# verdurin/pbdagcon

Hardware: AMD Instinct MI355X
Metric: consensus bases/sec (whole node) (higher is better)
Workload: dtype u8

## Files before the change

### pbdagcon_amd/csrc/dagcon_api.hip

```cpp
#include <hip/hip_runtime.h>
#include <algorithm>
#include <cstdarg>
#include <cstdio>
#include <cstdlib>
#include <cstring>
#include <string>
#include <chrono>
#include <vector>

#include "../../include/dagcon.h"
#include "dagcon_dev.h"
#include "k_build.hip.h"
#include "k_merge.hip.h"
#include "k_merge_q.hip.h"
#include "k_bestpath.hip.h"
#include "k_align.hip.h"
#include "k_align_panels.hip.h"
#include "k_place.hip.h"
#include "k_cigar.hip.h"
#include "k_cs.hip.h"

namespace {

struct DevBuf {
    void *p = nullptr;
    size_t cap = 0;
};

#define DQ_KMAX 52u
struct DgPlanIn { uint32_t T; uint64_t n_alns, sum_bb; uint32_t gcuts, max_segments, min_segment_len, seg_env, merge_q; };
struct DgPlan { uint32_t seg_max, seg_min, use_q, bp_max; };
static DgPlan dg_plan_pieces(const DgPlanIn &in) {
    DgPlan pl;
    const uint32_t T = in.T;
    pl.seg_min = in.min_segment_len;
    if (!pl.seg_min) pl.seg_min = (uint32_t)std::min<uint64_t>(768, std::max<uint64_t>(192, in.sum_bb / 8192));
    if (in.max_segments) pl.seg_max = in.max_segments > 64u ? 64u : in.max_segments;
    else if (in.seg_env) pl.seg_max = in.seg_env;
    else if (in.gcuts) pl.seg_max = 64;
    else { uint32_t sm = T ? 8192u / T : 8u; pl.seg_max = sm < 8u ? 8u : sm > 256u ? 256u : sm; }
    if (in.gcuts && !in.min_segment_len) pl.seg_min = 256;
    pl.use_q = 0;
    if (in.merge_q && !in.gcuts && pl.seg_max != 1) {
        const uint32_t slots = 1024u * DQ_WAVES;
        if (in.max_segments || in.seg_env) pl.use_q = 1;
        else if (T && in.n_alns <= (uint64_t)DQ_KMAX * T) {
            const uint64_t avail = std::min<uint64_t>(256, std::max<uint64_t>(1, in.sum_bb / T / 128));
            const uint64_t k = (uint64_t)T * avail / DQ_ROWS / slots;
            if (k >= 1 || (uint64_t)T * avail / DQ_ROWS * 10u >= 6u * slots) {
                const uint64_t sm = std::min<uint64_t>(avail, std::max<uint64_t>(k, 1) * slots * DQ_ROWS / T);
                if (sm >= 2) { pl.seg_max = (uint32_t)sm; pl.use_q = 1; }
            }
        }
    }
    if (pl.seg_max < 1) pl.seg_max = 1;
    if (pl.use_q && !in.min_segment_len) pl.seg_min = 128;
    pl.bp_max = pl.seg_max == 1 ? 1u : std::min(in.gcuts || T >= 256u ? 64u : (uint32_t)DG_BP_PIECES, 3u * pl.seg_max);
    if (pl.bp_max < 1) pl.bp_max = 1;
    return pl;
}

struct Ctx {
    dagcon_opts opts;
    int device = 0;
    hipStream_t stream = nullptr;
    hipEvent_t ev[5] = {nullptr, nullptr, nullptr, nullptr, nullptr};
    std::string err;
    bool uploaded = false, ran = false, fetched = false;

    uint32_t T = 0, A = 0;
    int bp_lane = 1, bl_stk = -1;
    uint32_t align_dropped = 0;
    uint32_t align_n = 0;
    std::vector<uint32_t> h_ends;
    int poison = 0;
    int fold = 1;
    int merge_q = 1, use_q = 0;
    uint32_t max_k = 0, max_tlen = 0;
    uint64_t sum_len = 0, sum_bb = 0, mat_cells = 0, blob_bytes = 0;
    bool have_bb = false;
    std::vector<uint32_t> h_tlen, h_aln_len, h_aln_start, h_aln_tgt;
    std::vector<uint64_t> h_aln_begin, h_aln_off, h_mat_base, h_bbv_base, h_bb_off, h_matc_base;
    std::vector<uint32_t> h_matc_stride;
    uint64_t matc_cells = 0;
    std::vector<uint8_t> h_tactive;
    std::vector<uint32_t> h_ch_base, h_ch_aln;
    std::vector<uint64_t> h_norm_off;
    std::vector<uint32_t> h_ck_base;
    uint64_t n_ckpt = 0;
    uint32_t emit_shift = 9;
    uint32_t n_chunks = 0;
    uint64_t tmp_main = 0, tmp_cap = 0;

    DevBuf d_tfail, d_q, d_t, d_aln_off, d_aln_len, d_aln_start, d_aln_tgt, d_tlen, d_aln_begin, d_tactive,
        d_bb, d_bb_off, d_mat_base, d_bbv_base, d_matc_base, d_matc_stride;
    DevBuf d_nmis, d_norm_off, d_n_lo, d_n_hi, d_n_start, d_n_ins, d_n_del, d_norm;
    DevBuf d_ch_aln, d_ch_base, d_ch_k0, d_ch_next, d_ch_w, d_ch_tb, d_ch_flag, d_ch_src, d_ch_out, d_ch_adv,
        d_n_lb, d_norm_tmp, d_ckpt, d_ck_base;
    DevBuf d_node_base, d_n_nodes, d_pool_base, d_pool_size, d_pool_top, d_t_nins;
    DevBuf d_matA, d_matD, d_matC, d_cov, d_gcount, d_gbase, d_bid;
    DevBuf d_nodes, d_best, d_queue, d_score, d_cns_tmp, d_bp_tt, d_score_b;
    DevBuf d_pool, d_stk, d_cuts, d_cuts_bp, d_bp_stat, d_bp_len, d_worklist, d_rd, d_pro_state, d_sh_cnt, d_seg_done, d_wl_first, d_queue0, d_bp_end, d_bp_ab, d_defer, d_cns_tmp0;
    DevBuf d_al[15];
    DevBuf d_pn[18];
    DevBuf d_pl[14];
    DevBuf d_cs[10];
    DevBuf d_cg[18];
    std::vector<uint8_t> h_cig_bad;
    std::string cig_err;
    DevBuf d_cns, d_cns_off, d_cns_len, d_seg_first, d_n_seg, d_seg_r0, d_seg_r1, d_st;
    DevBuf d_pos_tmp, d_pos_tmp0, d_pos;
    DevBuf d_sup_tmp, d_sup_tmp0, d_sup;

    uint64_t norm_cap = 0, node_cap = 0, pool_cap = 0, cns_cap = 0, seg_cap = 0;
    uint32_t stk_words = 4096, growth_pct = 100, seg_max = 8, bp_max = 16, seg_env = 0, seg_min = 768;
    uint32_t sh_log = 16;
    bool full_span = false;
    uint32_t gcuts = 1;
    uint32_t worklist_cap = 0, list_grid = 8192;

    DgStatus h_st;
    dagcon_timings tm;

    std::vector<uint64_t> r_seg_begin, r_seq_off, r_cns_off, r_seg_first;
    std::vector<int32_t> r_range0, r_range1, r_tmp0, r_tmp1;
    std::vector<uint32_t> r_seq_len, r_cns_len, r_n_seg, r_tfail;
    std::vector<int32_t> r_status;
    char *r_blob = nullptr;
    size_t r_blob_cap = 0;
    uint16_t *r_sup = nullptr;
    size_t r_sup_cap = 0;
    uint64_t r_sup_n = 0;
    std::vector<uint32_t> r_pos;
    bool pos_valid = false;
    bool sup_valid = false;

    std::vector<uint8_t> g_base, g_deleted, g_backbone;
    std::vector<int32_t> g_weight, g_cov, g_bbpos, g_out_dst, g_out_cnt, g_in_src;
    std::vector<uint32_t> g_out_begin, g_in_begin;
};

int fail(Ctx *c, int code, const char *fmt, ...) {
    char buf[512];
    va_list ap;
    va_start(ap, fmt);
    vsnprintf(buf, sizeof buf, fmt, ap);
    va_end(ap);
    if (c) c->err = buf;
    return code;
}

#define HIPCHK(c, call)                                                                    \
    do {                                                                                   \
        hipError_t _e = (call);                                                            \
        if (_e != hipSuccess)                                                              \
            return fail((c), DAGCON_ERR_HIP, "%s failed: %s (%s:%d)", #call,               \
                        hipGetErrorString(_e), __FILE__, __LINE__);                        \
    } while (0)

int ensure(Ctx *c, DevBuf &b, size_t bytes) {
    if (bytes == 0) bytes = 16;
    if (b.cap >= bytes) return DAGCON_OK;
    if (b.p) { (void)hipFree(b.p); b.p = nullptr; b.cap = 0; }
    size_t want = bytes + bytes / 16 + 256;
    const bool dbg = getenv("DAGCON_ALLOC_TIMING") != nullptr;
    const double t0 = dbg ? std::chrono::duration<double>(std::chrono::steady_clock::now().time_since_epoch()).count() : 0;
    hipError_t e = hipMalloc(&b.p, want);
    if (dbg) {
        const double dt = std::chrono::duration<double>(std::chrono::steady_clock::now().time_since_epoch()).count() - t0;
        if (dt > 0.005) fprintf(stderr, "dagcon: hipMalloc(%.1f MB) took %.1f ms\n", want / 1e6, dt * 1e3);
    }
    if (e != hipSuccess) {
        b.p = nullptr;
        return fail(c, DAGCON_ERR_WORKSPACE, "hipMalloc(%zu bytes) failed: %s", want, hipGetErrorString(e));
    }
    b.cap = want;
    return DAGCON_OK;
}

#define ENSURE(c, buf, bytes)                                \
    do {                                                     \
        int _r = ensure((c), (buf), (size_t)(bytes));        \
        if (_r != DAGCON_OK) return _r;                      \
    } while (0)

template <typename T>
int upload_vec(Ctx *c, DevBuf &b, const std::vector<T> &v) {
    ENSURE(c, b, v.size() * sizeof(T));
    if (!v.empty()) HIPCHK(c, hipMemcpyAsync(b.p, v.data(), v.size() * sizeof(T), hipMemcpyHostToDevice, c->stream));
    return DAGCON_OK;
}

void free_buf(DevBuf &b) {
    if (b.p) (void)hipFree(b.p);
    b.p = nullptr; b.cap = 0;
}

int ensure_arenas(Ctx *c) {
    ENSURE(c, c->d_norm, c->norm_cap * sizeof(uint16_t));
    ENSURE(c, c->d_nodes, c->node_cap * sizeof(DgNode));
    ENSURE(c, c->d_best, c->node_cap * 4);
    ENSURE(c, c->d_queue, c->node_cap * 4);
    ENSURE(c, c->d_score, c->node_cap * 8);
    ENSURE(c, c->d_bp_tt, c->node_cap * 4);
    if (c->gcuts) ENSURE(c, c->d_score_b, c->node_cap * 4);
    ENSURE(c, c->d_cns_tmp, c->node_cap);
    ENSURE(c, c->d_pool, c->pool_cap * 4);
    ENSURE(c, c->d_stk, std::max<uint64_t>((uint64_t)c->T * std::max(c->bp_max, c->seg_max), c->gcuts ? c->list_grid : 0) * c->stk_words * 4);
    if (c->gcuts) {
        ENSURE(c, c->d_worklist, (4ull + 3ull * c->worklist_cap) * 4);
        ENSURE(c, c->d_rd, (uint64_t)c->A * 16 + 16);
        ENSURE(c, c->d_pro_state, (uint64_t)c->T * 16 + 16);
        ENSURE(c, c->d_sh_cnt, (uint64_t)c->T * (2 + 2 * DG_SH_MAX) * 4 + 16);
        ENSURE(c, c->d_seg_done, (uint64_t)c->worklist_cap * (DG_SH_MAX + 1) * 4 + 16);
        ENSURE(c, c->d_wl_first, (uint64_t)c->T * 4 + 16);
        ENSURE(c, c->d_queue0, c->node_cap * 4);
        ENSURE(c, c->d_bp_end, (uint64_t)c->T * c->bp_max * 4 + 16);
        ENSURE(c, c->d_bp_ab, (uint64_t)c->T * c->bp_max * 16 + 16);
        ENSURE(c, c->d_defer, (uint64_t)c->T * (DG_DEFER_MAX + 1) * 4 + 16);
        ENSURE(c, c->d_cns_tmp0, c->node_cap);
    }
    ENSURE(c, c->d_cuts, (uint64_t)c->T * (c->seg_max + 2) * 4);
    ENSURE(c, c->d_cuts_bp, (uint64_t)c->T * (c->bp_max + 2) * 4);
    ENSURE(c, c->d_bp_stat, (uint64_t)c->T * c->bp_max * 8);
    ENSURE(c, c->d_bp_len, (uint64_t)c->T * c->bp_max * 4);
    ENSURE(c, c->d_cns, c->cns_cap);
    if (c->opts.flags & DAGCON_FLAG_BASE_SUPPORT) {
        ENSURE(c, c->d_sup_tmp, c->node_cap * 4);
        if (c->gcuts) ENSURE(c, c->d_sup_tmp0, c->node_cap * 4);
        ENSURE(c, c->d_sup, c->cns_cap * 4);
    }
    if (c->opts.flags & DAGCON_FLAG_BASE_POS) {
        ENSURE(c, c->d_pos_tmp, c->node_cap * 4);
        if (c->gcuts) ENSURE(c, c->d_pos_tmp0, c->node_cap * 4);
        ENSURE(c, c->d_pos, c->cns_cap * 4);
    }
    ENSURE(c, c->d_seg_r0, c->seg_cap * 4);
    ENSURE(c, c->d_seg_r1, c->seg_cap * 4);
    return DAGCON_OK;
}

void fill_params(Ctx *c, DgParams &p) {
    memset(&p, 0, sizeof p);
    p.q = (const uint8_t *)c->d_q.p; p.t = (const uint8_t *)c->d_t.p;
    p.aln_off = (const uint64_t *)c->d_aln_off.p;
    p.aln_len = (const uint32_t *)c->d_aln_len.p;
    p.aln_start = (const uint32_t *)c->d_aln_start.p;
    p.aln_tgt = (const uint32_t *)c->d_aln_tgt.p;
    p.tlen = (const uint32_t *)c->d_tlen.p;
    p.aln_begin = (const uint64_t *)c->d_aln_begin.p;
    p.tactive = (const uint8_t *)c->d_tactive.p; p.tfail = (uint32_t *)c->d_tfail.p;
    p.bb = c->have_bb ? (const uint8_t *)c->d_bb.p : nullptr;
    p.bb_off = (const uint64_t *)c->d_bb_off.p;
    p.mat_base = (const uint64_t *)c->d_mat_base.p;
    p.matc_base = (const uint64_t *)c->d_matc_base.p; p.matc_stride = (const uint32_t *)c->d_matc_stride.p;
    p.bbv_base = (const uint64_t *)c->d_bbv_base.p;
    p.T = c->T; p.A = c->A;
    p.trim = c->opts.trim; p.min_len = c->opts.min_len;
    p.min_weight = c->opts.min_weight < 0 ? (int32_t)c->opts.min_cov : c->opts.min_weight;
    p.flags = c->opts.flags;
    p.max_k = c->max_k; p.max_tlen = c->max_tlen;
    p.nmis = (uint32_t *)c->d_nmis.p; p.norm_off = (uint64_t *)c->d_norm_off.p;
    p.n_lo = (uint32_t *)c->d_n_lo.p; p.n_hi = (uint32_t *)c->d_n_hi.p;
    p.n_start = (uint32_t *)c->d_n_start.p; p.n_ins = (uint32_t *)c->d_n_ins.p;
    p.n_del = (uint32_t *)c->d_n_del.p;
    p.norm = (uint16_t *)c->d_norm.p; p.norm_cap = c->norm_cap;
    p.ch_aln = (const uint32_t *)c->d_ch_aln.p; p.ch_base = (const uint32_t *)c->d_ch_base.p;
    p.n_chunks = c->n_chunks;
    p.ch_k0 = (uint32_t *)c->d_ch_k0.p; p.ch_next = (uint32_t *)c->d_ch_next.p;
    p.ch_w = (uint32_t *)c->d_ch_w.p; p.ch_tb = (uint32_t *)c->d_ch_tb.p;
    p.ch_flag = (uint32_t *)c->d_ch_flag.p; p.ch_src = (uint64_t *)c->d_ch_src.p;
    p.ch_out = (uint32_t *)c->d_ch_out.p; p.ch_adv = (uint32_t *)c->d_ch_adv.p;
    p.n_lb = (uint32_t *)c->d_n_lb.p; p.norm_tmp = (uint16_t *)c->d_norm_tmp.p;
    p.tmp_main = c->tmp_main; p.tmp_cap = c->tmp_cap;
    p.ckpt = (uint32_t *)c->d_ckpt.p; p.ck_base = (const uint32_t *)c->d_ck_base.p; p.emit_shift = c->emit_shift;
    p.node_base = (uint64_t *)c->d_node_base.p; p.n_nodes = (uint32_t *)c->d_n_nodes.p;
    p.pool_base = (uint64_t *)c->d_pool_base.p; p.pool_size = (uint32_t *)c->d_pool_size.p;
    p.pool_top = (uint32_t *)c->d_pool_top.p; p.t_nins = (uint32_t *)c->d_t_nins.p;
    p.matA = (uint32_t *)c->d_matA.p; p.matD = (uint32_t *)c->d_matD.p; p.matC = (uint32_t *)c->d_matC.p;
    p.cov = (int32_t *)c->d_cov.p; p.gcount = (uint32_t *)c->d_gcount.p;
    p.gbase = (uint32_t *)c->d_gbase.p; p.bid = (uint32_t *)c->d_bid.p;
    p.nodes = (DgNode *)c->d_nodes.p; p.best = (int32_t *)c->d_best.p;
    p.queue = (int32_t *)c->d_queue.p; p.score = (float2 *)c->d_score.p; p.bp_tt = (float *)c->d_bp_tt.p;
    p.cns_tmp = (uint8_t *)c->d_cns_tmp.p; p.node_cap = c->node_cap;
    p.pool = (uint32_t *)c->d_pool.p; p.pool_cap = c->pool_cap;
    p.stk = (int32_t *)c->d_stk.p; p.stk_words = c->stk_words; p.growth_pct = c->growth_pct;
    p.score_b = (float *)c->d_score_b.p;
    p.bp_lane = c->bp_lane >= 2 || (c->bp_lane && (uint64_t)c->T * c->bp_max >= 32768ull) ? 1u : 0u; p.bl_stk = c->bl_stk >= 0 && c->bl_stk < DG_BL_STK ? (uint32_t)c->bl_stk : (uint32_t)DG_BL_STK;
    p.emit_scan = c->max_k <= 64u ? 1u : 0u;
    p.fold = (c->fold && !(c->opts.flags & DAGCON_FLAG_STOP_AFTER_BUILD)) ? 1u : 0u;
    p.q_kmax = c->use_q && !c->opts.max_segments && !c->seg_env && c->max_k > DQ_KMAX ? DQ_KMAX : 0u;
    p.bp_seg_min = (c->seg_min + 2u) / 3u;
    p.seg_max = c->seg_max; p.seg_min = c->seg_min; p.cuts = (uint32_t *)c->d_cuts.p; p.bp_max = c->bp_max; p.cuts_bp = (uint32_t *)c->d_cuts_bp.p; p.bp_stat = (float *)c->d_bp_stat.p; p.bp_len = (uint32_t *)c->d_bp_len.p;
    p.gcuts = c->gcuts; p.sh_log = c->sh_log;
    p.rd_s = (uint32_t *)c->d_rd.p; p.rd_e = p.rd_s + c->A; p.rd_lead = p.rd_e + c->A; p.rd_trail = p.rd_lead + c->A;
    p.pro_state = (uint32_t *)c->d_pro_state.p; p.sh_cnt = (uint32_t *)c->d_sh_cnt.p;
    p.queue0 = (int32_t *)c->d_queue0.p; p.bp_end = (uint32_t *)c->d_bp_end.p; p.bp_ab = (float *)c->d_bp_ab.p;
    p.defer = (uint32_t *)c->d_defer.p; p.cns_tmp0 = (uint8_t *)c->d_cns_tmp0.p;
    p.seg_done = (uint32_t *)c->d_seg_done.p; p.wl_first = (uint32_t *)c->d_wl_first.p;
    p.worklist = (uint32_t *)c->d_worklist.p; p.worklist_cap = c->worklist_cap;
    p.cns = (uint8_t *)c->d_cns.p; p.cns_cap = c->cns_cap;
    p.cns_off = (uint64_t *)c->d_cns_off.p; p.cns_len = (uint32_t *)c->d_cns_len.p;
    p.seg_first = (uint64_t *)c->d_seg_first.p; p.n_seg = (uint32_t *)c->d_n_seg.p;
    p.seg_r0 = (int32_t *)c->d_seg_r0.p; p.seg_r1 = (int32_t *)c->d_seg_r1.p;
    p.seg_cap = c->seg_cap;
    p.st = (DgStatus *)c->d_st.p;
    if (c->opts.flags & DAGCON_FLAG_BASE_SUPPORT) {
        p.sup_tmp = (uint32_t *)c->d_sup_tmp.p; p.sup_tmp0 = (uint32_t *)c->d_sup_tmp0.p;
        p.sup_w = (uint16_t *)c->d_sup.p; p.sup_d = p.sup_w + c->cns_cap;
    }
    if (c->opts.flags & DAGCON_FLAG_BASE_POS) {
        p.pos_tmp = (uint32_t *)c->d_pos_tmp.p; p.pos_tmp0 = (uint32_t *)c->d_pos_tmp0.p; p.pos_out = (uint32_t *)c->d_pos.p;
    }
}

void launch_normalize(Ctx *c, const DgParams &p) {
    hipStream_t s = c->stream;
    if (c->A == 0) return;
    (void)hipMemsetAsync(c->d_ckpt.p, 0xFF, c->n_ckpt * 4, s);
    hipLaunchKernelGGL((k_norm_chunk<DG_NW, 64, false>), dim3((c->n_chunks + 63) / 64), dim3(64), 0, s, p);
    hipLaunchKernelGGL((k_norm_chunk<DG_NW_BIG, 32, true>), dim3((c->n_chunks + 31) / 32), dim3(32), 0, s, p);
    hipLaunchKernelGGL(k_norm_scan, dim3((c->A + 63) / 64), dim3(64), 0, s, p);
    hipLaunchKernelGGL(k_norm_finish2, dim3((c->n_chunks + 3) / 4), dim3(256), 0, s, p);
    hipLaunchKernelGGL(k_normalize_slow, dim3((c->A + 63) / 64), dim3(64), 0, s, p);
}

int launch_all(Ctx *c) {
    int r = ensure_arenas(c);
    if (r != DAGCON_OK) return r;
    DgParams p;
    fill_params(c, p);
    hipStream_t s = c->stream;
    if (c->poison & 8) {
        DevBuf *work[] = {&c->d_nmis, &c->d_n_lo, &c->d_n_hi, &c->d_n_start, &c->d_n_ins, &c->d_n_del, &c->d_ch_k0, &c->d_ch_next, &c->d_ch_w,
                          &c->d_ch_tb, &c->d_ch_flag, &c->d_ch_src, &c->d_ch_out, &c->d_ch_adv, &c->d_n_lb, &c->d_norm_tmp, &c->d_ckpt,
                          &c->d_node_base, &c->d_n_nodes, &c->d_pool_base, &c->d_pool_size, &c->d_pool_top, &c->d_t_nins, &c->d_cov, &c->d_gcount,
                          &c->d_gbase, &c->d_bid, &c->d_best, &c->d_queue, &c->d_score, &c->d_cns_tmp, &c->d_bp_tt, &c->d_stk, &c->d_cuts,
                          &c->d_cuts_bp, &c->d_bp_stat, &c->d_bp_len, &c->d_rd, &c->d_pro_state, &c->d_sh_cnt, &c->d_wl_first,
                          &c->d_queue0, &c->d_bp_end, &c->d_bp_ab, &c->d_defer, &c->d_cns_tmp0, &c->d_cns, &c->d_cns_off, &c->d_seg_first,
                          &c->d_seg_r0, &c->d_seg_r1, &c->d_worklist, &c->d_seg_done, &c->d_sup_tmp, &c->d_sup_tmp0, &c->d_sup, &c->d_pos_tmp, &c->d_pos_tmp0, &c->d_pos};
        for (DevBuf *b : work)
            if (b->p && b->cap) HIPCHK(c, hipMemsetAsync(b->p, 0xEE, b->cap, s));
    }
    HIPCHK(c, hipMemsetAsync(c->d_st.p, 0, sizeof(DgStatus), s));
    HIPCHK(c, hipMemsetAsync(c->d_tfail.p, 0, (size_t)c->T * 4 + 4, s));
    HIPCHK(c, hipMemsetAsync(c->d_cns_len.p, 0, (size_t)c->T * 4, s));
    HIPCHK(c, hipMemsetAsync(c->d_n_seg.p, 0, (size_t)c->T * 4, s));
    if (c->matc_cells) HIPCHK(c, hipMemsetAsync(c->d_matC.p, 0, c->matc_cells * 4, s));
    if (c->poison) {
        if ((c->poison & 1) && c->d_matA.p) { HIPCHK(c, hipMemsetAsync(c->d_matA.p, 0xEE, c->d_matA.cap, s)); HIPCHK(c, hipMemsetAsync(c->d_matD.p, 0xEE, c->d_matD.cap, s)); }
        if ((c->poison & 2) && c->d_nodes.p) { HIPCHK(c, hipMemsetAsync(c->d_nodes.p, 0xEE, c->d_nodes.cap, s)); HIPCHK(c, hipMemsetAsync(c->d_pool.p, 0xEE, c->d_pool.cap, s)); }
        if ((c->poison & 4) && c->d_score_b.p) HIPCHK(c, hipMemsetAsync(c->d_score_b.p, 0xEE, c->d_score_b.cap, s));
        if ((c->poison & 4) && c->d_norm.p) HIPCHK(c, hipMemsetAsync(c->d_norm.p, 0xEE, c->d_norm.cap, s));
    }
    HIPCHK(c, hipEventRecord(c->ev[0], s));
    launch_normalize(c, p);
    HIPCHK(c, hipEventRecord(c->ev[1], s));
    hipLaunchKernelGGL(k_carve, dim3(1), dim3(1024), 0, s, p);
    if (c->T > 0) {
        const uint32_t rows4 = (c->max_tlen + 2 + 4 * DG_LPW - 1) / (4 * DG_LPW);
        if (c->gcuts && c->A > 0) hipLaunchKernelGGL(k_readspan, dim3((c->A + 63) / 64), dim3(64), 0, s, p);
        if (p.emit_scan) hipLaunchKernelGGL(k_gsum, dim3(c->T, (c->max_tlen + 2 + 255) / 256), dim3(256), 0, s, p);
        else hipLaunchKernelGGL(k_groups, dim3(c->T, (c->max_tlen + 2 + 31) / 32), dim3(256), 0, s, p);
        hipLaunchKernelGGL(k_gscan, dim3(c->T), dim3(1024), 0, s, p);
        if (c->A > 0)
            hipLaunchKernelGGL(k_emit, dim3(c->T, (c->max_k + DG_ERPW - 1) / DG_ERPW, ((c->max_tlen + 2) >> c->emit_shift) + 1),
                               dim3(64), 0, s, p);
        const size_t lds = (size_t)4 * 2 * (c->max_k + 2) * sizeof(int32_t);
        if (lds > 65536)
            HIPCHK(c, hipFuncSetAttribute((const void *)k_lists, hipFuncAttributeMaxDynamicSharedMemorySize, (int)lds));
        hipLaunchKernelGGL(k_lists, dim3(c->T, rows4), dim3(256), lds, s, p);
    }
    HIPCHK(c, hipEventRecord(c->ev[2], s));
    if (c->T > 0 && !(c->opts.flags & DAGCON_FLAG_STOP_AFTER_BUILD)) {
        if (c->gcuts) {
            HIPCHK(c, hipMemsetAsync(c->d_worklist.p, 0, 16, s));
            HIPCHK(c, hipMemsetAsync(c->d_seg_done.p, 0, (size_t)c->worklist_cap * (DG_SH_MAX + 1) * 4, s));
            hipLaunchKernelGGL(k_merge_pro, dim3(c->T), dim3(64), 0, s, p);
            hipLaunchKernelGGL(k_cuts2, dim3(c->T), dim3(64), 0, s, p);
            hipLaunchKernelGGL(k_merge_list, dim3(c->list_grid), dim3(64), 0, s, p);
            hipLaunchKernelGGL(k_merge_fin, dim3(c->T), dim3(64), 0, s, p);
        } else {
            hipLaunchKernelGGL(k_cuts, dim3(c->T), dim3(64), 0, s, p);
            if (c->use_q) {
                hipLaunchKernelGGL(k_merge_q, dim3((c->T * c->seg_max + DQ_ROWS - 1u) / DQ_ROWS), dim3(64), 0, s, p);
                if (p.q_kmax) hipLaunchKernelGGL(k_merge, dim3(c->T * c->seg_max), dim3(64), 0, s, p);
            } else hipLaunchKernelGGL(k_merge, dim3(c->T * c->seg_max), dim3(64), 0, s, p);
        }
    }
    HIPCHK(c, hipEventRecord(c->ev[3], s));
    if (c->T > 0 && !(c->opts.flags & (DAGCON_FLAG_STOP_AFTER_BUILD | DAGCON_FLAG_STOP_AFTER_MERGE))) {
        const bool sup = (c->opts.flags & DAGCON_FLAG_BASE_SUPPORT) != 0;
        const bool pos = (c->opts.flags & DAGCON_FLAG_BASE_POS) != 0;
#define DG_BP_LAUNCH(K, GRID)                                                                          \
        do {                                                                                           \
            if (sup && pos) hipLaunchKernelGGL((K<true, true>), GRID, dim3(64), 0, s, p);              \
            else if (sup) hipLaunchKernelGGL((K<true, false>), GRID, dim3(64), 0, s, p);               \
            else if (pos) hipLaunchKernelGGL((K<false, true>), GRID, dim3(64), 0, s, p);               \
            else hipLaunchKernelGGL((K<false, false>), GRID, dim3(64), 0, s, p);                       \
        } while (0)
        hipLaunchKernelGGL(k_bp_terms, dim3(c->T, 16), dim3(256), 0, s, p);
        if (c->gcuts) {
            hipLaunchKernelGGL(k_bp_xtree, dim3(c->T), dim3(64), 0, s, p);
            hipLaunchKernelGGL(k_bp_sweep_ab, dim3(c->T * c->bp_max), dim3(64), 0, s, p);
            hipLaunchKernelGGL(k_bp_comb, dim3(c->T), dim3(64), 0, s, p);
            hipLaunchKernelGGL(k_bp_abs, dim3(c->T * c->bp_max), dim3(256), 0, s, p);
            hipLaunchKernelGGL(k_bp_choose, dim3(c->T * c->bp_max), dim3(256), 0, s, p);
            hipLaunchKernelGGL(k_bp_sweep_abs_g, dim3(c->T * c->bp_max), dim3(64), 0, s, p);
            hipLaunchKernelGGL(k_bp_defer, dim3(c->T), dim3(64), 0, s, p);
            DG_BP_LAUNCH(k_bp_walk_g, dim3(c->T * c->bp_max));
        } else {
            if (p.bp_lane) hipLaunchKernelGGL(k_bp_sweep_l, dim3((c->T * c->bp_max + 7u) / 8u), dim3(64), 0, s, p);
            hipLaunchKernelGGL(k_bp_sweep, dim3(c->T * c->bp_max), dim3(64), 0, s, p);
            hipLaunchKernelGGL(k_bp_check, dim3(c->T), dim3(64), 0, s, p);
            if (p.bp_lane) DG_BP_LAUNCH(k_bp_walk_r, dim3((c->T * c->bp_max + 7u) / 8u));
            else DG_BP_LAUNCH(k_bp_walk, dim3(c->T * c->bp_max));
        }
        DG_BP_LAUNCH(k_bp_join, dim3(c->T));
#undef DG_BP_LAUNCH
    }
    HIPCHK(c, hipEventRecord(c->ev[4], s));
    HIPCHK(c, hipGetLastError());
    return DAGCON_OK;
}

}

extern "C" {

int dagcon_abi_version(void) { return DAGCON_ABI_VERSION; }

void dagcon_default_opts(dagcon_opts *o) {
    if (!o) return;
    memset(o, 0, sizeof *o);
    o->min_cov = 6; o->min_len = 500; o->trim = 50; o->min_weight = -1; o->device = 0; o->flags = 0;
}

const char *dagcon_last_error(const dagcon_ctx *ctx) {
    return ctx ? reinterpret_cast<const Ctx *>(ctx)->err.c_str() : "null context";
}

int dagcon_create(const dagcon_opts *opts, dagcon_ctx **out) {
    if (!opts || !out) return DAGCON_ERR_INVALID_ARG;
    *out = nullptr;
    int ndev = 0;
    if (hipGetDeviceCount(&ndev) != hipSuccess || ndev <= 0) return DAGCON_ERR_NO_DEVICE;
    if (opts->device < 0 || opts->device >= ndev) return DAGCON_ERR_NO_DEVICE;
    if (opts->flags & ~DAGCON_FLAGS_ALL) return DAGCON_ERR_UNSUPPORTED;
    {
        hipDeviceProp_t prop;
        if (hipGetDeviceProperties(&prop, opts->device) != hipSuccess || strncmp(prop.gcnArchName, "gfx950", 6) != 0)
            return DAGCON_ERR_NO_DEVICE;
    }
    Ctx *c = new Ctx();
    c->opts = *opts;
    c->device = opts->device;
    if (const char *e = getenv("DAGCON_EMIT_SHIFT")) {
        const int v = atoi(e);
        if (v >= 4 && v <= 20) c->emit_shift = (uint32_t)v;
    }
    if (const char *e = getenv("DAGCON_MERGE_SEGS")) {
        const int v = atoi(e);
        if (v >= 1 && v <= 64) c->seg_env = (uint32_t)v;
    }
    if (const char *e = getenv("DAGCON_FOLD")) c->fold = atoi(e) != 0;
    if (const char *e = getenv("DAGCON_POISON")) c->poison = atoi(e);
    if (const char *e = getenv("DAGCON_BP_LANE")) c->bp_lane = atoi(e);
    if (const char *e = getenv("DAGCON_BP_LANE_STACK")) c->bl_stk = atoi(e);
    if (const char *e = getenv("DAGCON_MERGE_Q")) c->merge_q = atoi(e) != 0;
    memset(&c->tm, 0, sizeof c->tm);
    memset(&c->h_st, 0, sizeof c->h_st);
    if (hipSetDevice(c->device) != hipSuccess || hipStreamCreateWithFlags(&c->stream, hipStreamNonBlocking) != hipSuccess) {
        delete c;
        return DAGCON_ERR_NO_DEVICE;
    }
    for (auto &e : c->ev)
        if (hipEventCreate(&e) != hipSuccess) { delete c; return DAGCON_ERR_HIP; }
    if (ensure(c, c->d_st, sizeof(DgStatus)) != DAGCON_OK) { delete c; return DAGCON_ERR_WORKSPACE; }
    *out = reinterpret_cast<dagcon_ctx *>(c);
    return DAGCON_OK;
}

void dagcon_destroy(dagcon_ctx *ctx) {
    if (!ctx) return;
    Ctx *c = reinterpret_cast<Ctx *>(ctx);
    (void)hipSetDevice(c->device);
    if (c->stream) (void)hipStreamSynchronize(c->stream);
    if (c->r_blob) (void)hipHostFree(c->r_blob);
    if (c->r_sup) (void)hipHostFree(c->r_sup);
    DevBuf *all[] = {&c->d_q, &c->d_t, &c->d_aln_off, &c->d_aln_len, &c->d_aln_start, &c->d_aln_tgt,
                     &c->d_tlen, &c->d_aln_begin, &c->d_tactive, &c->d_tfail, &c->d_bb, &c->d_bb_off, &c->d_mat_base, &c->d_matc_base, &c->d_matc_stride,
                     &c->d_bbv_base, &c->d_nmis, &c->d_norm_off, &c->d_n_lo, &c->d_n_hi, &c->d_n_start, &c->d_ch_aln, &c->d_ch_base, &c->d_ch_k0, &c->d_ch_next, &c->d_ch_w, &c->d_ch_tb, &c->d_ch_flag, &c->d_ch_src, &c->d_ch_out, &c->d_ch_adv, &c->d_n_lb, &c->d_norm_tmp, &c->d_ckpt, &c->d_ck_base,
                     &c->d_n_ins, &c->d_n_del, &c->d_norm, &c->d_node_base, &c->d_n_nodes,
                     &c->d_pool_base, &c->d_pool_size, &c->d_pool_top, &c->d_t_nins, &c->d_matA, &c->d_matD,
                     &c->d_matC, &c->d_cov, &c->d_gcount, &c->d_gbase, &c->d_bid, &c->d_nodes,
                     &c->d_best, &c->d_queue, &c->d_score, &c->d_cns_tmp, &c->d_bp_tt, &c->d_score_b, &c->d_pool, &c->d_stk, &c->d_cuts, &c->d_cuts_bp, &c->d_bp_stat, &c->d_bp_len, &c->d_worklist, &c->d_rd, &c->d_pro_state, &c->d_sh_cnt, &c->d_seg_done, &c->d_wl_first, &c->d_queue0, &c->d_bp_end, &c->d_bp_ab, &c->d_defer, &c->d_cns_tmp0, &c->d_cns,
                     &c->d_cns_off, &c->d_cns_len, &c->d_seg_first, &c->d_n_seg, &c->d_seg_r0, &c->d_seg_r1,
                     &c->d_st, &c->d_sup_tmp, &c->d_sup_tmp0, &c->d_sup, &c->d_pos_tmp, &c->d_pos_tmp0, &c->d_pos};
    for (DevBuf *b : all) free_buf(*b);
    for (DevBuf &b : c->d_al) free_buf(b);
    for (DevBuf &b : c->d_pn) free_buf(b);
    for (DevBuf &b : c->d_pl) free_buf(b);
    for (DevBuf &b : c->d_cg) free_buf(b);
    for (DevBuf &b : c->d_cs) free_buf(b);
    for (auto &e : c->ev) if (e) (void)hipEventDestroy(e);
    if (c->stream) (void)hipStreamDestroy(c->stream);
    delete c;
}

static int upload_impl(dagcon_ctx *ctx, const dagcon_batch *b, const void *dev_q, const void *dev_t) {
    if (!ctx || !b) return DAGCON_ERR_INVALID_ARG;
    Ctx *c = reinterpret_cast<Ctx *>(ctx);
    c->uploaded = c->ran = c->fetched = false;
    c->sup_valid = c->pos_valid = false;
    c->h_cig_bad.clear();
    const uint32_t T = b->n_targets;
    if (T && (!b->tlen || !b->aln_begin)) return fail(c, DAGCON_ERR_INVALID_ARG, "tlen/aln_begin is NULL");
    const uint64_t A_all = T ? b->aln_begin[T] : 0;
    if (A_all && (!b->aln_start || !b->aln_off || !b->aln_len || ((!b->qstr || !b->tstr) && !(dev_q && dev_t))))
        return fail(c, DAGCON_ERR_INVALID_ARG, "alignment arrays are NULL");
    if (b->backbone && !b->backbone_off) return fail(c, DAGCON_ERR_INVALID_ARG, "backbone_off is NULL");
    HIPCHK(c, hipSetDevice(c->device));

    c->T = T;
    c->h_tlen.assign(b->tlen, b->tlen + T);
    c->h_aln_begin.assign(T + 1, 0);
    c->h_tactive.assign(T, 0);
    c->h_mat_base.assign(T, 0);
    c->h_matc_base.assign(T, 0); c->h_matc_stride.assign(T, 0); c->matc_cells = 0;
    c->h_bbv_base.assign(T, 0);
    c->h_bb_off.assign(T, 0);
    c->h_aln_len.clear(); c->h_aln_start.clear(); c->h_aln_tgt.clear(); c->h_aln_off.clear();
    c->max_k = 0; c->max_tlen = 0; c->sum_len = 0; c->sum_bb = 0; c->mat_cells = 0;
    c->have_bb = b->backbone != nullptr;
    uint64_t bb_bytes = 0, n_whole = 0;
    const uint64_t min_cov = c->opts.min_cov;
    for (uint32_t t = 0; t < T; t++) {
        const uint64_t ab = b->aln_begin[t], ae = b->aln_begin[t + 1];
        if (ae < ab) return fail(c, DAGCON_ERR_INVALID_ARG, "aln_begin not monotone at target %u", t);
        const uint64_t k_all = ae - ab;
        const bool active = k_all > 0 && k_all >= min_cov;
        c->h_aln_begin[t] = c->h_aln_len.size();
        if (!active) continue;
        if (b->tlen[t] > 0x3FFFFFFFu) return fail(c, DAGCON_ERR_UNSUPPORTED, "tlen of target %u too large", t);
        c->h_tactive[t] = 1;
        for (uint64_t a = ab; a < ae; a++) {
            const uint32_t len = b->aln_len[a];
            if (b->aln_off[a] > b->blob_bytes || len > b->blob_bytes - b->aln_off[a])
                return fail(c, DAGCON_ERR_INVALID_ARG, "alignment %llu runs past the blob", (unsigned long long)a);
            if (len < c->opts.min_len) continue;
            c->h_aln_len.push_back(len);
            c->h_aln_start.push_back(b->aln_start[a]);
            c->h_aln_off.push_back(b->aln_off[a]);
            c->h_aln_tgt.push_back(t);
            c->sum_len += len;
            n_whole += len >= b->tlen[t] && b->aln_start[a] == 1u;
        }
        const uint64_t k = c->h_aln_len.size() - c->h_aln_begin[t];
        if (k > DAGCON_MAX_COVERAGE)
            return fail(c, DAGCON_ERR_UNSUPPORTED, "target %u has %llu alignments (max %u)", t,
                        (unsigned long long)k, DAGCON_MAX_COVERAGE);
        c->max_k = std::max<uint32_t>(c->max_k, (uint32_t)k);
        c->max_tlen = std::max(c->max_tlen, b->tlen[t]);
        if ((uint64_t)b->tlen[t] + 2 > 4ull * 65535ull)
            return fail(c, DAGCON_ERR_UNSUPPORTED, "tlen of target %u exceeds %u", t, 4u * 65535u - 2u);
        c->h_mat_base[t] = c->mat_cells;
        c->mat_cells += ((uint64_t)b->tlen[t] + 2) * k;
        c->h_matc_stride[t] = (b->tlen[t] + 2 + 7) & ~7u;
        c->h_matc_base[t] = c->matc_cells;
        c->matc_cells += (uint64_t)c->h_matc_stride[t] * k;
        c->h_bbv_base[t] = c->sum_bb;
        c->sum_bb += ((uint64_t)b->tlen[t] + 2 + 3) & ~3ull;
        if (c->have_bb) {
            c->h_bb_off[t] = b->backbone_off[t];
            bb_bytes = std::max<uint64_t>(bb_bytes, b->backbone_off[t] + b->tlen[t]);
        }
    }
    c->full_span = n_whole == (uint64_t)c->h_aln_len.size();
    c->gcuts = c->full_span ? 0u : 1u;
    if (const char *e = getenv("DAGCON_GCUTS")) c->gcuts = atoi(e) ? 1u : 0u;
    {
        DgPlanIn pi;
        pi.T = T; pi.n_alns = c->h_aln_len.size(); pi.sum_bb = c->sum_bb; pi.gcuts = c->gcuts;
        pi.max_segments = c->opts.max_segments; pi.min_segment_len = c->opts.min_segment_len;
        pi.seg_env = c->seg_env; pi.merge_q = c->merge_q ? 1u : 0u;
        const DgPlan pl = dg_plan_pieces(pi);
        c->seg_max = pl.seg_max; c->seg_min = pl.seg_min; c->use_q = (int)pl.use_q; c->bp_max = pl.bp_max;
    }
    if (const char *e = getenv("DAGCON_BP_SEGS")) { const int v = atoi(e); if (v >= 1 && v <= 64) c->bp_max = (uint32_t)v; }
    {
        const uint64_t pieces = std::max<uint64_t>(1, (uint64_t)T * std::max(c->bp_max, c->seg_max));
        const uint32_t fit = (uint32_t)std::min<uint64_t>(4096, (512ull << 20) / pieces);
        const uint32_t base = std::max(256u, fit);
        if (c->stk_words < base || (uint64_t)c->stk_words * pieces > (1024ull << 20)) c->stk_words = base;
    }
    if (c->gcuts) c->worklist_cap = std::max<uint32_t>(c->worklist_cap, (uint32_t)std::min<uint64_t>((uint64_t)T * c->seg_max + 64, 0x0FFFFFFFull));
    c->h_aln_begin[T] = c->h_aln_len.size();
    if (c->h_aln_len.size() > 0xFFFFFFF0ull) return fail(c, DAGCON_ERR_UNSUPPORTED, "too many alignments");
    c->A = (uint32_t)c->h_aln_len.size();
    c->blob_bytes = b->blob_bytes;
    c->h_ch_base.assign((size_t)c->A + 1, 0);
    c->h_ch_aln.clear();
    for (uint32_t a = 0; a < c->A; a++) {
        const uint32_t nw = std::max<uint32_t>(1u, (c->h_aln_len[a] + DG_NCH - 1) / DG_NCH);
        c->h_ch_base[a] = (uint32_t)c->h_ch_aln.size();
        if (c->h_ch_aln.size() + nw > 0xFFFFFFF0ull) return fail(c, DAGCON_ERR_UNSUPPORTED, "too many alignment columns");
        c->h_ch_aln.insert(c->h_ch_aln.end(), nw, a);
    }
    c->h_norm_off.assign((size_t)c->A, 0);
    {
        uint64_t top = 0;
        for (uint32_t a = 0; a < c->A; a++) { c->h_norm_off[a] = top; top += (2ull * c->h_aln_len[a] + 7ull) & ~7ull; }
        c->norm_cap = std::max<uint64_t>(c->norm_cap, top + 64);
    }
    c->h_ck_base.assign((size_t)c->A, 0);
    c->n_ckpt = 0;
    for (uint32_t a = 0; a < c->A; a++) {
        c->h_ck_base[a] = (uint32_t)c->n_ckpt;
        c->n_ckpt += (((uint64_t)c->h_tlen[c->h_aln_tgt[a]] + 2) >> c->emit_shift) + 1;
        if (c->n_ckpt > 0xFFFFFFF0ull) return fail(c, DAGCON_ERR_UNSUPPORTED, "too many alignment columns");
    }
    c->h_ch_base[c->A] = (uint32_t)c->h_ch_aln.size();
    c->n_chunks = (uint32_t)c->h_ch_aln.size();
    c->tmp_main = (2ull * b->blob_bytes + 8ull * c->n_chunks + 15ull) & ~7ull;
    c->tmp_cap = c->tmp_main + std::max<uint64_t>(c->tmp_main / 16, 1ull << 20);

    ENSURE(c, c->d_q, b->blob_bytes);
    ENSURE(c, c->d_t, b->blob_bytes);
    if (b->blob_bytes && !(dev_q == c->d_q.p && dev_t == c->d_t.p)) {
        HIPCHK(c, hipMemcpyAsync(c->d_q.p, dev_q ? dev_q : b->qstr, b->blob_bytes, dev_q ? hipMemcpyDeviceToDevice : hipMemcpyHostToDevice, c->stream));
        HIPCHK(c, hipMemcpyAsync(c->d_t.p, dev_t ? dev_t : b->tstr, b->blob_bytes, dev_t ? hipMemcpyDeviceToDevice : hipMemcpyHostToDevice, c->stream));
    }
    if (c->have_bb) {
        ENSURE(c, c->d_bb, bb_bytes);
        if (bb_bytes) HIPCHK(c, hipMemcpyAsync(c->d_bb.p, b->backbone, bb_bytes, hipMemcpyHostToDevice, c->stream));
    }
    int r;
    if ((r = upload_vec(c, c->d_aln_off, c->h_aln_off))) return r;
    if ((r = upload_vec(c, c->d_aln_len, c->h_aln_len))) return r;
    if ((r = upload_vec(c, c->d_aln_start, c->h_aln_start))) return r;
    if ((r = upload_vec(c, c->d_aln_tgt, c->h_aln_tgt))) return r;
    if ((r = upload_vec(c, c->d_tlen, c->h_tlen))) return r;
    if ((r = upload_vec(c, c->d_aln_begin, c->h_aln_begin))) return r;
    if ((r = upload_vec(c, c->d_tactive, c->h_tactive))) return r;
    if ((r = upload_vec(c, c->d_bb_off, c->h_bb_off))) return r;
    if ((r = upload_vec(c, c->d_mat_base, c->h_mat_base))) return r;
    if ((r = upload_vec(c, c->d_matc_base, c->h_matc_base))) return r;
    if ((r = upload_vec(c, c->d_matc_stride, c->h_matc_stride))) return r;
    if ((r = upload_vec(c, c->d_bbv_base, c->h_bbv_base))) return r;
    if ((r = upload_vec(c, c->d_ch_base, c->h_ch_base))) return r;
    if ((r = upload_vec(c, c->d_ch_aln, c->h_ch_aln))) return r;
    if ((r = upload_vec(c, c->d_ck_base, c->h_ck_base))) return r;
    if ((r = upload_vec(c, c->d_norm_off, c->h_norm_off))) return r;
    ENSURE(c, c->d_ckpt, c->n_ckpt * 4);

    const size_t A4 = (size_t)c->A * 4, T4 = (size_t)T * 4;
    ENSURE(c, c->d_nmis, A4);
    ENSURE(c, c->d_n_lo, A4); ENSURE(c, c->d_n_hi, A4); ENSURE(c, c->d_n_start, A4);
    ENSURE(c, c->d_n_ins, A4); ENSURE(c, c->d_n_del, A4); ENSURE(c, c->d_n_lb, A4);
    {
        const size_t C4 = (size_t)c->n_chunks * 4;
        ENSURE(c, c->d_ch_k0, C4); ENSURE(c, c->d_ch_next, C4); ENSURE(c, c->d_ch_w, C4); ENSURE(c, c->d_ch_tb, C4);
        ENSURE(c, c->d_ch_flag, C4); ENSURE(c, c->d_ch_src, 2 * C4); ENSURE(c, c->d_ch_out, C4); ENSURE(c, c->d_ch_adv, C4);
        ENSURE(c, c->d_norm_tmp, c->tmp_cap * sizeof(uint16_t));
    }
    ENSURE(c, c->d_node_base, (size_t)T * 8); ENSURE(c, c->d_n_nodes, T4);
    ENSURE(c, c->d_pool_base, (size_t)T * 8); ENSURE(c, c->d_pool_size, T4); ENSURE(c, c->d_pool_top, T4);
    ENSURE(c, c->d_t_nins, T4); ENSURE(c, c->d_tfail, T4 + 4);
    ENSURE(c, c->d_matA, c->mat_cells * 4); ENSURE(c, c->d_matD, c->mat_cells * 4);
    ENSURE(c, c->d_matC, c->matc_cells * 4 + 256);
    ENSURE(c, c->d_cov, c->sum_bb * 4); ENSURE(c, c->d_gcount, c->sum_bb * 4);
    ENSURE(c, c->d_gbase, c->sum_bb * 4); ENSURE(c, c->d_bid, c->sum_bb * 4);
    ENSURE(c, c->d_cns_off, (size_t)T * 8); ENSURE(c, c->d_cns_len, T4);
    ENSURE(c, c->d_seg_first, (size_t)T * 8); ENSURE(c, c->d_n_seg, T4);

    c->node_cap = std::max<uint64_t>(c->node_cap, c->sum_bb + c->sum_len / 7 + 1024);
    c->pool_cap = std::max<uint64_t>(c->pool_cap, 8ull * c->node_cap + 80ull * c->sum_bb + 1024ull * T);
    c->cns_cap = std::max<uint64_t>(c->cns_cap, c->sum_bb + c->sum_bb / 4 + 1024);
    c->seg_cap = std::max<uint64_t>(c->seg_cap, (uint64_t)T * 4 + 1024);
    if ((r = ensure_arenas(c))) return r;
    HIPCHK(c, hipStreamSynchronize(c->stream));
    c->uploaded = true;
    c->tm.reruns = 0;
    return DAGCON_OK;
}

int dagcon_upload(dagcon_ctx *ctx, const dagcon_batch *b) { return upload_impl(ctx, b, nullptr, nullptr); }

int dagcon_run(dagcon_ctx *ctx) {
    if (!ctx) return DAGCON_ERR_INVALID_ARG;
    Ctx *c = reinterpret_cast<Ctx *>(ctx);
    if (!c->uploaded) return fail(c, DAGCON_ERR_STATE, "dagcon_run before dagcon_upload");
    HIPCHK(c, hipSetDevice(c->device));
    int r = launch_all(c);
    if (r != DAGCON_OK) return r;
    c->ran = true; c->fetched = false;
    if (const char *e = getenv("DAGCON_DUMP")) {
        const uint32_t t = (uint32_t)atoi(e);
        const char *path = strchr(e, ':');
        if (path && t < c->T) {
            HIPCHK(c, hipStreamSynchronize(c->stream));
            uint64_t nb = 0, pb = 0;
            uint32_t hdr[4] = {0, c->bp_max, 0, c->seg_max};
            (void)hipMemcpy(&nb, (uint64_t *)c->d_node_base.p + t, 8, hipMemcpyDeviceToHost);
            (void)hipMemcpy(&pb, (uint64_t *)c->d_pool_base.p + t, 8, hipMemcpyDeviceToHost);
            (void)hipMemcpy(&hdr[0], (uint32_t *)c->d_n_nodes.p + t, 4, hipMemcpyDeviceToHost);
            (void)hipMemcpy(&hdr[2], (uint32_t *)c->d_pool_top.p + t, 4, hipMemcpyDeviceToHost);
            std::vector<uint32_t> cuts(c->bp_max + 2), pool(hdr[2]), best(hdr[0]);
            std::vector<DgNode> nd(hdr[0]);
            std::vector<float> sc(2 * (size_t)hdr[0]);
            (void)hipMemcpy(cuts.data(), (uint32_t *)c->d_cuts_bp.p + (uint64_t)t * (c->bp_max + 2), cuts.size() * 4, hipMemcpyDeviceToHost);
            (void)hipMemcpy(nd.data(), (DgNode *)c->d_nodes.p + nb, nd.size() * sizeof(DgNode), hipMemcpyDeviceToHost);
            (void)hipMemcpy(pool.data(), (uint32_t *)c->d_pool.p + pb, pool.size() * 4, hipMemcpyDeviceToHost);
            (void)hipMemcpy(sc.data(), (float *)c->d_score.p + 2 * nb, sc.size() * 4, hipMemcpyDeviceToHost);
            (void)hipMemcpy(best.data(), (uint32_t *)c->d_best.p + nb, best.size() * 4, hipMemcpyDeviceToHost);
            if (FILE *f = fopen(path + 1, "wb")) {
                fwrite(hdr, 4, 4, f); fwrite(cuts.data(), 4, cuts.size(), f); fwrite(nd.data(), sizeof(DgNode), nd.size(), f);
                fwrite(pool.data(), 4, pool.size(), f); fwrite(sc.data(), 4, sc.size(), f); fwrite(best.data(), 4, best.size(), f);
                uint32_t nl = 0;
                std::vector<uint32_t> wl;
                if (c->gcuts && c->d_worklist.p) {
                    (void)hipMemcpy(&nl, c->d_worklist.p, 4, hipMemcpyDeviceToHost);
                    if (nl > c->worklist_cap) nl = c->worklist_cap;
                    wl.resize(3 * (size_t)nl);
                    if (nl) (void)hipMemcpy(wl.data(), (uint32_t *)c->d_worklist.p + 4, wl.size() * 4, hipMemcpyDeviceToHost);
                }
                fwrite(&nl, 4, 1, f);
                if (nl) fwrite(wl.data(), 4, wl.size(), f);
                fclose(f);
            }
        }
    }
    return DAGCON_OK;
}

int dagcon_sync(dagcon_ctx *ctx) {
    if (!ctx) return DAGCON_ERR_INVALID_ARG;
    Ctx *c = reinterpret_cast<Ctx *>(ctx);
    HIPCHK(c, hipSetDevice(c->device));
    HIPCHK(c, hipStreamSynchronize(c->stream));
    return DAGCON_OK;
}

static hipError_t d2h(Ctx *c, void *dst, const void *src, size_t bytes) {
    hipError_t e = hipMemcpyAsync(dst, src, bytes, hipMemcpyDeviceToHost, c->stream);
    return e != hipSuccess ? e : hipStreamSynchronize(c->stream);
}

static int read_status(Ctx *c) {
    HIPCHK(c, hipStreamSynchronize(c->stream));
    HIPCHK(c, d2h(c, &c->h_st, c->d_st.p, sizeof(DgStatus)));
    return DAGCON_OK;
}

int dagcon_fetch(dagcon_ctx *ctx, dagcon_results *res) {
    if (!ctx || !res) return DAGCON_ERR_INVALID_ARG;
    Ctx *c = reinterpret_cast<Ctx *>(ctx);
    if (!c->ran) return fail(c, DAGCON_ERR_STATE, "dagcon_fetch before dagcon_run");
    HIPCHK(c, hipSetDevice(c->device));
    int r;
    for (int attempt = 0;; attempt++) {
        if ((r = read_status(c))) return r;
        const uint32_t f = c->h_st.err_flags;
        if (f == 0) break;
        if (f & DG_E_TARGET_MASK)
            return fail(c, DAGCON_ERR_INTERNAL, "unexpected batch-level flag 0x%x", f);
        if (attempt >= 6) return fail(c, DAGCON_ERR_WORKSPACE, "workspace still too small after %d re-runs (flags 0x%x)", attempt, f);
        if (f & DG_E_NORM_OVF) c->norm_cap = c->h_st.norm_top + 1024;
        if (f & DG_E_NODE_OVF) c->node_cap = c->h_st.node_need + 1024;
        if (f & DG_E_POOL_OVF) c->pool_cap = c->h_st.pool_need + 1024;
        if (f & DG_E_POOL_TGT) c->growth_pct *= 3;
        if (f & DG_E_STACK) c->stk_words *= 4;
        if (f & DG_E_LIST_OVF) c->worklist_cap *= 4;
        if (f & DG_E_LOG_OVF) c->sh_log *= 2;
        if (f & DG_E_OUT_OVF) {
            c->cns_cap = std::max<uint64_t>(c->cns_cap, c->h_st.cns_top + 1024);
            c->seg_cap = std::max<uint64_t>(c->seg_cap, c->h_st.seg_top + 1024);
        }
        c->tm.reruns++;
        if ((r = launch_all(c))) return r;
    }
    float ms = 0;
    HIPCHK(c, hipEventElapsedTime(&ms, c->ev[0], c->ev[4])); c->tm.ms_total = ms;
    HIPCHK(c, hipEventElapsedTime(&ms, c->ev[0], c->ev[1])); c->tm.ms_normalize = ms;
    HIPCHK(c, hipEventElapsedTime(&ms, c->ev[1], c->ev[2])); c->tm.ms_build = ms;
    HIPCHK(c, hipEventElapsedTime(&ms, c->ev[2], c->ev[3])); c->tm.ms_merge = ms;
    HIPCHK(c, hipEventElapsedTime(&ms, c->ev[3], c->ev[4])); c->tm.ms_bestpath = ms;

    const uint32_t T = c->T;
    c->r_tfail.assign(T, 0); c->r_status.assign(T, DAGCON_OK);
    if (T) HIPCHK(c, d2h(c, c->r_tfail.data(), c->d_tfail.p, (size_t)T * 4));
    uint32_t n_failed = 0;
    c->err.clear();
    for (uint32_t t = 0; t < T; t++) {
        const uint32_t f = c->r_tfail[t];
        if (!f) continue;
        const int code = (f & (DG_E_BADCHAR | DG_E_NONCONF)) ? DAGCON_ERR_NONCONFORMING
                       : (f & DG_E_TOO_BIG) ? DAGCON_ERR_UNSUPPORTED : DAGCON_ERR_INTERNAL;
        c->r_status[t] = code;
        if (!n_failed++) {
            if (f & DG_E_BADCHAR) fail(c, code, "target %u: an alignment holds a byte outside printable ASCII", t);
            else if (f & DG_E_NONCONF) fail(c, code, "target %u: an alignment (after the min_len filter) leaves the backbone: start < 1 or target bases past tlen", t);
            else if (f & DG_E_TOO_BIG) fail(c, code, "target %u too large (more than 2^25 - 3 vertices or 2^30 pool words)", t);
            else fail(c, code, "device invariant violated in target %u", t);
        }
    }
    for (uint32_t t = 0; t < T && !c->h_cig_bad.empty(); t++) {
        if (!c->h_cig_bad[t] || c->r_status[t] != DAGCON_OK) continue;
        c->r_status[t] = DAGCON_ERR_NONCONFORMING;
        if (!n_failed++) c->err = c->cig_err;
    }
    const uint64_t nseg = c->h_st.seg_top, nb = c->h_st.cns_top;
    c->r_cns_off.assign(T, 0); c->r_cns_len.assign(T, 0); c->r_seg_first.assign(T, 0); c->r_n_seg.assign(T, 0);
    c->r_tmp0.assign(nseg, 0); c->r_tmp1.assign(nseg, 0);
    if (c->r_blob_cap < nb + 1) {
        if (c->r_blob) (void)hipHostFree(c->r_blob);
        c->r_blob = nullptr; c->r_blob_cap = 0;
        const size_t want = (size_t)(nb + 1) + (size_t)(nb / 8) + 4096;
        HIPCHK(c, hipHostMalloc((void **)&c->r_blob, want, hipHostMallocDefault));
        c->r_blob_cap = want;
    }
    c->r_blob[nb] = 0;
    const bool full = !(c->opts.flags & (DAGCON_FLAG_STOP_AFTER_BUILD | DAGCON_FLAG_STOP_AFTER_MERGE));
    if (T && full) {
        HIPCHK(c, d2h(c, c->r_cns_off.data(), c->d_cns_off.p, (size_t)T * 8));
        HIPCHK(c, d2h(c, c->r_cns_len.data(), c->d_cns_len.p, (size_t)T * 4));
        HIPCHK(c, d2h(c, c->r_seg_first.data(), c->d_seg_first.p, (size_t)T * 8));
        HIPCHK(c, d2h(c, c->r_n_seg.data(), c->d_n_seg.p, (size_t)T * 4));
        if (nseg) {
            HIPCHK(c, d2h(c, c->r_tmp0.data(), c->d_seg_r0.p, nseg * 4));
            HIPCHK(c, d2h(c, c->r_tmp1.data(), c->d_seg_r1.p, nseg * 4));
        }
        if (nb) HIPCHK(c, d2h(c, c->r_blob, c->d_cns.p, nb));
    }
    c->sup_valid = c->pos_valid = false;
    if (full && (c->opts.flags & DAGCON_FLAG_BASE_SUPPORT)) {
        if (c->r_sup_cap < nb + 1) {
            if (c->r_sup) (void)hipHostFree(c->r_sup);
            c->r_sup = nullptr; c->r_sup_cap = 0;
            const size_t want = (size_t)(nb + 1) + (size_t)(nb / 8) + 4096;
            HIPCHK(c, hipHostMalloc((void **)&c->r_sup, want * 4, hipHostMallocDefault));
            c->r_sup_cap = want;
        }
        if (nb) {
            HIPCHK(c, hipMemcpyAsync(c->r_sup, c->d_sup.p, nb * 2, hipMemcpyDeviceToHost, c->stream));
            HIPCHK(c, d2h(c, c->r_sup + nb, (const uint16_t *)c->d_sup.p + c->cns_cap, nb * 2));
        }
        c->r_sup_n = nb;
        c->sup_valid = true;
    }
    if (full && (c->opts.flags & DAGCON_FLAG_BASE_POS)) {
        c->r_pos.resize(nb + 1);
        if (nb) HIPCHK(c, d2h(c, c->r_pos.data(), c->d_pos.p, nb * 4));
        c->pos_valid = true;
    }
    c->r_seg_begin.assign(T + 1, 0);
    c->r_range0.clear(); c->r_range1.clear(); c->r_seq_off.clear(); c->r_seq_len.clear();
    uint64_t bases = 0;
    for (uint32_t t = 0; t < T; t++) {
        c->r_seg_begin[t] = c->r_range0.size();
        if (!full || !c->h_tactive[t] || c->r_tfail[t]) continue;
        for (uint32_t i = 0; i < c->r_n_seg[t]; i++) {
            const uint64_t s = c->r_seg_first[t] + i;
            const int32_t r0 = c->r_tmp0[s], r1 = c->r_tmp1[s];
            c->r_range0.push_back(r0); c->r_range1.push_back(r1);
            c->r_seq_off.push_back(c->r_cns_off[t] + (uint64_t)r0);
            c->r_seq_len.push_back((uint32_t)(r1 - r0));
            bases += (uint64_t)(r1 - r0);
        }
    }
    c->r_seg_begin[T] = c->r_range0.size();
    c->tm.consensus_bases = bases;
    c->tm.algorithmic_bytes = 2ull * c->sum_len + bases;
    c->tm.n_alignments = c->A;
    c->tm.n_columns = c->h_st.n_columns;
    c->tm.n_nodes = c->h_st.node_need;
    c->tm.merge_segments = c->h_st.n_mseg;
    res->n_targets = T;
    res->n_segments = c->r_range0.size();
    res->seg_begin = c->r_seg_begin.data();
    res->range0 = c->r_range0.data(); res->range1 = c->r_range1.data();
    res->seq_off = c->r_seq_off.data(); res->seq_len = c->r_seq_len.data();
    res->seq_blob = c->r_blob; res->seq_bytes = nb;
    res->target_status = c->r_status.data(); res->n_failed = n_failed;
    c->fetched = true;
    return DAGCON_OK;
}

int dagcon_fetch_support(dagcon_ctx *ctx, dagcon_support *out) {
    if (!ctx || !out) return DAGCON_ERR_INVALID_ARG;
    Ctx *c = reinterpret_cast<Ctx *>(ctx);
    if (!(c->opts.flags & DAGCON_FLAG_BASE_SUPPORT))
        return fail(c, DAGCON_ERR_STATE, "dagcon_fetch_support on a context created without DAGCON_FLAG_BASE_SUPPORT");
    if (!c->sup_valid)
        return fail(c, DAGCON_ERR_STATE, "dagcon_fetch_support without the results of a consensus (no fetch yet, or stopped before bestPath)");
    out->n = c->r_sup_n;
    out->weight = c->r_sup;
    out->depth = c->r_sup + c->r_sup_n;
    return DAGCON_OK;
}

int dagcon_fetch_positions(dagcon_ctx *ctx, const uint32_t **pos, uint64_t *n) {
    if (!ctx || !pos || !n) return DAGCON_ERR_INVALID_ARG;
    Ctx *c = reinterpret_cast<Ctx *>(ctx);
    if (!(c->opts.flags & DAGCON_FLAG_BASE_POS))
        return fail(c, DAGCON_ERR_STATE, "dagcon_fetch_positions on a context created without DAGCON_FLAG_BASE_POS");
    if (!c->pos_valid)
        return fail(c, DAGCON_ERR_STATE, "dagcon_fetch_positions without the results of a consensus (no fetch yet, or stopped before bestPath)");
    *pos = c->r_pos.data();
    *n = c->r_pos.size() - 1;
    return DAGCON_OK;
}

int dagcon_debug_counters(dagcon_ctx *ctx, unsigned long long *out8) {
    if (!ctx || !out8) return DAGCON_ERR_INVALID_ARG;
    Ctx *c = reinterpret_cast<Ctx *>(ctx);
    HIPCHK(c, hipSetDevice(c->device));
    HIPCHK(c, hipStreamSynchronize(c->stream));
    DgStatus st;
    HIPCHK(c, d2h(c, &st, c->d_st.p, sizeof st));
    for (int i = 0; i < 16; i++) out8[i] = st.dbg[i];
    return DAGCON_OK;
}

uint32_t dagcon_align_dropped(dagcon_ctx *ctx) {
    return ctx ? reinterpret_cast<Ctx *>(ctx)->align_dropped : 0u;
}

int dagcon_debug_plan(uint32_t n_targets, uint64_t n_alignments, uint64_t sum_positions, uint32_t partial_span,
                      uint32_t max_segments, uint32_t min_segment_len, uint32_t out4[4]) {
    if (!out4) return DAGCON_ERR_INVALID_ARG;
    DgPlanIn pi;
    pi.T = n_targets; pi.n_alns = n_alignments; pi.sum_bb = sum_positions; pi.gcuts = partial_span ? 1u : 0u;
    pi.max_segments = max_segments; pi.min_segment_len = min_segment_len; pi.seg_env = 0; pi.merge_q = 1;
    const DgPlan pl = dg_plan_pieces(pi);
    out4[0] = pl.seg_max; out4[1] = pl.seg_min; out4[2] = pl.use_q; out4[3] = pl.bp_max;
    return DAGCON_OK;
}

int dagcon_get_timings(dagcon_ctx *ctx, dagcon_timings *out) {
    if (!ctx || !out) return DAGCON_ERR_INVALID_ARG;
    Ctx *c = reinterpret_cast<Ctx *>(ctx);
    if (!c->ran) return fail(c, DAGCON_ERR_STATE, "no run to report");
    if (!c->fetched) {
        HIPCHK(c, hipSetDevice(c->device));
        HIPCHK(c, hipStreamSynchronize(c->stream));
        float ms = 0;
        HIPCHK(c, hipEventElapsedTime(&ms, c->ev[0], c->ev[4])); c->tm.ms_total = ms;
        HIPCHK(c, hipEventElapsedTime(&ms, c->ev[0], c->ev[1])); c->tm.ms_normalize = ms;
        HIPCHK(c, hipEventElapsedTime(&ms, c->ev[1], c->ev[2])); c->tm.ms_build = ms;
        HIPCHK(c, hipEventElapsedTime(&ms, c->ev[2], c->ev[3])); c->tm.ms_merge = ms;
        HIPCHK(c, hipEventElapsedTime(&ms, c->ev[3], c->ev[4])); c->tm.ms_bestpath = ms;
    }
    *out = c->tm;
    return DAGCON_OK;
}

int dagcon_consensus(dagcon_ctx *ctx, const dagcon_batch *batch, dagcon_results *results) {
    int r = dagcon_upload(ctx, batch);
    if (r != DAGCON_OK) return r;
    if ((r = dagcon_run(ctx)) != DAGCON_OK) return r;
    return dagcon_fetch(ctx, results);
}

static int normalize_impl(Ctx *c, dagcon_ctx *ctx, uint32_t n, const uint32_t *aln_start,
                          const uint64_t *aln_off, const uint32_t *aln_len, const char *qstr,
                          const char *tstr, uint64_t blob_bytes, const uint64_t *out_off, char *qout,
                          char *tout, uint32_t *out_len, uint32_t *out_start) {
    std::vector<uint32_t> tl(1, 0u);
    std::vector<uint64_t> ab = {0, n};
    dagcon_batch b;
    memset(&b, 0, sizeof b);
    b.n_targets = 1; b.tlen = tl.data(); b.aln_begin = ab.data();
    b.aln_start = aln_start; b.aln_off = aln_off; b.aln_len = aln_len;
    b.qstr = qstr; b.tstr = tstr; b.blob_bytes = blob_bytes;
    int r = dagcon_upload(ctx, &b);
    if (r != DAGCON_OK) return r;
    for (int attempt = 0;; attempt++) {
        DgParams p;
        fill_params(c, p);
        p.flags |= DG_F_A1_ONLY;
        HIPCHK(c, hipMemsetAsync(c->d_st.p, 0, sizeof(DgStatus), c->stream));
        HIPCHK(c, hipMemsetAsync(c->d_tfail.p, 0, (size_t)c->T * 4 + 4, c->stream));
        launch_normalize(c, p);
        HIPCHK(c, hipGetLastError());
        if ((r = read_status(c))) return r;
        if ((c->h_st.err_flags & DG_E_NORM_OVF) && attempt < 3) {
            c->norm_cap = c->h_st.norm_top + 1024;
            if ((r = ensure_arenas(c))) return r;
            continue;
        }
        break;
    }
    if (c->h_st.err_flags & DG_E_BADCHAR)
        return fail(c, DAGCON_ERR_NONCONFORMING, "alignment %u holds a byte outside printable ASCII", c->h_st.bad_aln);
    if (c->h_st.err_flags) return fail(c, DAGCON_ERR_INTERNAL, "normalize failed (flags 0x%x)", c->h_st.err_flags);
    std::vector<uint64_t> noff(n);
    std::vector<uint32_t> lo(n), hi(n), st(n);
    if (n) {
        HIPCHK(c, d2h(c, noff.data(), c->d_norm_off.p, (size_t)n * 8));
        HIPCHK(c, d2h(c, lo.data(), c->d_n_lo.p, (size_t)n * 4));
        HIPCHK(c, d2h(c, hi.data(), c->d_n_hi.p, (size_t)n * 4));
        HIPCHK(c, d2h(c, st.data(), c->d_n_start.p, (size_t)n * 4));
    }
    std::vector<uint16_t> cols;
    for (uint32_t a = 0; a < n; a++) {
        const uint32_t m = hi[a] - lo[a];
        cols.resize(m);
        if (m) HIPCHK(c, d2h(c, cols.data(), (const uint16_t *)c->d_norm.p + noff[a] + lo[a], (size_t)m * 2));
        for (uint32_t i = 0; i < m; i++) {
            qout[out_off[a] + i] = (char)(cols[i] & 0xff);
            tout[out_off[a] + i] = (char)(cols[i] >> 8);
        }
        out_len[a] = m;
        out_start[a] = st[a];
    }
    return DAGCON_OK;
}

int dagcon_normalize(dagcon_ctx *ctx, uint32_t n, const uint32_t *aln_start, const uint64_t *aln_off,
                     const uint32_t *aln_len, const char *qstr, const char *tstr, uint64_t blob_bytes,
                     uint32_t trim, uint32_t flags, const uint64_t *out_off, char *qout, char *tout,
                     uint32_t *out_len, uint32_t *out_start) {
    if (!ctx) return DAGCON_ERR_INVALID_ARG;
    Ctx *c = reinterpret_cast<Ctx *>(ctx);
    if (n && (!aln_start || !aln_off || !aln_len || !qstr || !tstr || !out_off || !qout || !tout || !out_len || !out_start))
        return fail(c, DAGCON_ERR_INVALID_ARG, "NULL argument");
    if (n > DAGCON_MAX_COVERAGE)
        return fail(c, DAGCON_ERR_UNSUPPORTED, "dagcon_normalize takes at most %u alignments per call", DAGCON_MAX_COVERAGE);
    const dagcon_opts saved = c->opts;
    c->opts.min_cov = 0; c->opts.min_len = 0; c->opts.trim = trim;
    c->opts.flags = flags & DAGCON_FLAG_RAW_ALIGNMENTS;
    const int r = normalize_impl(c, ctx, n, aln_start, aln_off, aln_len, qstr, tstr, blob_bytes, out_off,
                                 qout, tout, out_len, out_start);
    c->opts = saved;
    c->uploaded = false; c->ran = false;
    return r;
}

extern "C++" {
template <bool LOCAL>
static void launch_align_band(uint32_t cells, uint32_t nk, hipStream_t s, const DgAlignParams &ap) {
    switch (cells) {
        case 2: hipLaunchKernelGGL((k_align_band<2, LOCAL>), dim3(nk), dim3(64), 0, s, ap); break;
        case 4: hipLaunchKernelGGL((k_align_band<4, LOCAL>), dim3(nk), dim3(64), 0, s, ap); break;
        case 6: hipLaunchKernelGGL((k_align_band<6, LOCAL>), dim3(nk), dim3(64), 0, s, ap); break;
        case 8: hipLaunchKernelGGL((k_align_band<8, LOCAL>), dim3(nk), dim3(64), 0, s, ap); break;
        case 12: hipLaunchKernelGGL((k_align_band<12, LOCAL>), dim3(nk), dim3(64), 0, s, ap); break;
        default: hipLaunchKernelGGL((k_align_band<16, LOCAL>), dim3(nk), dim3(64), 0, s, ap); break;
    }
}
}

static int align_device(Ctx *c, uint32_t n, const uint64_t *q_off, const uint32_t *q_len,
                        const uint64_t *t_off, const uint32_t *t_len, const char *q_blob, uint64_t q_bytes,
                        const char *t_blob, uint64_t t_bytes, const uint64_t *out_off, uint32_t *aln_len, uint64_t *out_bytes_ret) {
    HIPCHK(c, hipSetDevice(c->device));
    const bool local = (c->opts.flags & DAGCON_FLAG_LOCAL_ALIGN) != 0;
    c->align_n = 0;
    uint64_t out_bytes = 0;
    std::vector<uint64_t> dir_off(n);
    for (uint32_t a = 0; a < n; a++) {
        if (q_off[a] > q_bytes || q_len[a] > q_bytes - q_off[a] || t_off[a] > t_bytes || t_len[a] > t_bytes - t_off[a])
            return fail(c, DAGCON_ERR_INVALID_ARG, "pair %u runs past its blob", a);
        if ((uint64_t)q_len[a] + t_len[a] > 0x7FFFFFF0ull) return fail(c, DAGCON_ERR_UNSUPPORTED, "pair %u too long", a);
        out_bytes = std::max<uint64_t>(out_bytes, out_off[a] + (uint64_t)q_len[a] + t_len[a]);
    }
    DevBuf &dq = c->d_al[0], &dt = c->d_al[1], &dqo = c->d_al[2], &dto = c->d_al[3], &dql = c->d_al[4], &dtl = c->d_al[5],
           &doo = c->d_al[6], &dqa = c->d_al[7], &dta = c->d_al[8], &dlen = c->d_al[9], &ddir = c->d_al[10], &ddo = c->d_al[11];
    ENSURE(c, dq, q_bytes); ENSURE(c, dt, t_bytes);
    ENSURE(c, dqo, (size_t)n * 8); ENSURE(c, dto, (size_t)n * 8); ENSURE(c, dql, (size_t)n * 4); ENSURE(c, dtl, (size_t)n * 4);
    ENSURE(c, doo, (size_t)n * 8); ENSURE(c, dqa, out_bytes); ENSURE(c, dta, out_bytes); ENSURE(c, dlen, (size_t)n * 4);
    ENSURE(c, ddo, (size_t)n * 8);
    DevBuf &dend = c->d_al[14];
    if (local) ENSURE(c, dend, (size_t)n * 16);
    hipStream_t s = c->stream;
    HIPCHK(c, hipMemcpyAsync(dq.p, q_blob, q_bytes, hipMemcpyHostToDevice, s));
    HIPCHK(c, hipMemcpyAsync(dt.p, t_blob, t_bytes, hipMemcpyHostToDevice, s));
    HIPCHK(c, hipMemcpyAsync(dqo.p, q_off, (size_t)n * 8, hipMemcpyHostToDevice, s));
    HIPCHK(c, hipMemcpyAsync(dto.p, t_off, (size_t)n * 8, hipMemcpyHostToDevice, s));
    HIPCHK(c, hipMemcpyAsync(dql.p, q_len, (size_t)n * 4, hipMemcpyHostToDevice, s));
    HIPCHK(c, hipMemcpyAsync(dtl.p, t_len, (size_t)n * 4, hipMemcpyHostToDevice, s));
    HIPCHK(c, hipMemcpyAsync(doo.p, out_off, (size_t)n * 8, hipMemcpyHostToDevice, s));
    uint64_t budget_rows = (6ull << 30) / 256ull;
    {
        size_t mfree = 0, mtotal = 0;
        if (hipMemGetInfo(&mfree, &mtotal) == hipSuccess) {
            const uint64_t have = (uint64_t)mfree + (uint64_t)ddir.cap;
            budget_rows = std::min<uint64_t>(16ull << 30, std::max<uint64_t>(1ull << 30, have / 4)) / 256ull;
        }
    }
    if (const char *e = getenv("DAGCON_ALIGN_GB")) { const long long v = atoll(e); if (v >= 1 && v <= 200) budget_rows = ((uint64_t)v << 30) / 256ull; }
    if (const char *e = getenv("DAGCON_ALIGN_ROWS")) { const long long v = atoll(e); if (v >= 1) budget_rows = (uint64_t)v; }
    const bool t_dbg = getenv("DAGCON_ALIGN_TIMING") != nullptr;
    if (t_dbg) HIPCHK(c, hipStreamSynchronize(s));
    double t_grp = std::chrono::duration<double>(std::chrono::steady_clock::now().time_since_epoch()).count();
    DevBuf &didx = c->d_al[12], &dhw = c->d_al[13];
    ENSURE(c, didx, (size_t)n * 4); ENSURE(c, dhw, (size_t)n * 4);
    std::vector<uint32_t> todo(n), halfw(n), order(n);
    for (uint32_t a = 0; a < n; a++) todo[a] = a;
    DgAlignParams ap;
    ap.q = (const uint8_t *)dq.p; ap.t = (const uint8_t *)dt.p;
    ap.q_off = (const uint64_t *)dqo.p; ap.t_off = (const uint64_t *)dto.p;
    ap.q_len = (const uint32_t *)dql.p; ap.t_len = (const uint32_t *)dtl.p;
    ap.out_off = (const uint64_t *)doo.p; ap.qaln = (uint8_t *)dqa.p; ap.taln = (uint8_t *)dta.p;
    ap.aln_len = (uint32_t *)dlen.p; ap.dir_off = (const uint64_t *)ddo.p; ap.halfw = (const uint32_t *)dhw.p;
    ap.ends = local ? (uint32_t *)dend.p : nullptr;
    {
        std::vector<uint32_t> ad, rest;
        for (uint32_t a = 0; a < n; a++) (dg_align_halfwidth_first(q_len[a], t_len[a]) > DG_AL_WA ? ad : rest).push_back(a);
        if (getenv("DAGCON_ALIGN_STATIC")) { rest.insert(rest.end(), ad.begin(), ad.end()); ad.clear(); }
        std::stable_sort(ad.begin(), ad.end(), [&](uint32_t x, uint32_t y) { return q_len[x] > q_len[y]; });
        uint64_t all_rows = 0;
        for (uint32_t a : ad) all_rows += dg_align_rows_adapt(q_len[a], t_len[a]);
        const uint64_t ngrp = std::max<uint64_t>(1, (all_rows + budget_rows - 1) / budget_rows);
        const uint64_t grp_rows = std::min<uint64_t>(budget_rows, all_rows / ngrp + 1 + (all_rows / ngrp) / 64);
        size_t first = 0;
        while (first < ad.size()) {
            uint64_t rows = 0;
            size_t cnt = 0;
            while (first + cnt < ad.size()) {
                const uint32_t a = ad[first + cnt];
                const uint64_t r = dg_align_rows_adapt(q_len[a], t_len[a]);
                if (cnt && rows + r > grp_rows) break;
                dir_off[a] = rows;
                rows += r; cnt++;
            }
            ENSURE(c, ddir, rows * 256ull);
            ap.dirs = (uint32_t *)ddir.p;
            HIPCHK(c, hipMemcpyAsync(ddo.p, dir_off.data(), (size_t)n * 8, hipMemcpyHostToDevice, s));
            HIPCHK(c, hipMemcpyAsync((uint32_t *)didx.p + first, ad.data() + first, cnt * 4, hipMemcpyHostToDevice, s));
            ap.idx = (const uint32_t *)didx.p + first; ap.n = (uint32_t)cnt; ap.first_pass = 1u;
            if (local) hipLaunchKernelGGL(k_align_adapt<true>, dim3((uint32_t)cnt), dim3(64), 0, s, ap);
            else hipLaunchKernelGGL(k_align_adapt<false>, dim3((uint32_t)cnt), dim3(64), 0, s, ap);
            HIPCHK(c, hipGetLastError());
            HIPCHK(c, hipStreamSynchronize(s));
            if (t_dbg) {
                const double now = std::chrono::duration<double>(std::chrono::steady_clock::now().time_since_epoch()).count();
                fprintf(stderr, "dagcon_align: following band, group of %zu pairs, %.1f MB of directions: %.2f ms\n", cnt, rows * 256.0 / 1e6, (now - t_grp) * 1e3);
                t_grp = now;
            }
            first += cnt;
        }
        if (!ad.empty()) {
            HIPCHK(c, d2h(c, aln_len, dlen.p, (size_t)n * 4));
            size_t back = 0;
            for (uint32_t a : ad) if (aln_len[a] == DG_AL_RETRY) { rest.push_back(a); back++; }
            if (t_dbg) fprintf(stderr, "dagcon_align: %zu of %zu pairs go on to the static bands\n", back, ad.size());
        }
        std::sort(rest.begin(), rest.end());
        todo.swap(rest);
    }
    for (int pass = 0; pass < 2 && !todo.empty(); pass++) {
        for (uint32_t a : todo) halfw[a] = pass == 0 ? dg_align_halfwidth_first(q_len[a], t_len[a]) : dg_align_halfwidth(q_len[a], t_len[a]);
        HIPCHK(c, hipMemcpyAsync(dhw.p, halfw.data(), (size_t)n * 4, hipMemcpyHostToDevice, s));
        static const uint32_t kinds[6] = {2, 4, 6, 8, 12, 16};
        size_t first = 0;
        while (first < todo.size()) {
            uint64_t rows = 0;
            size_t cnt = 0;
            while (first + cnt < todo.size()) {
                const uint32_t a = todo[first + cnt];
                const uint64_t r = dg_align_rows(q_len[a], t_len[a], dg_align_cells(halfw[a]));
                if (cnt && rows + r > budget_rows) break;
                dir_off[a] = rows;
                rows += r; cnt++;
            }
            ENSURE(c, ddir, rows * 256ull);
            ap.dirs = (uint32_t *)ddir.p;
            HIPCHK(c, hipMemcpyAsync(ddo.p, dir_off.data(), (size_t)n * 8, hipMemcpyHostToDevice, s));
            size_t fill = 0;
            for (int k = 0; k < 6; k++) {
                for (int fin = 0; fin < 2; fin++) {
                    const size_t k0 = fill;
                    for (size_t x = 0; x < cnt; x++) {
                        const uint32_t a = todo[first + x];
                        const bool is_final = pass == 1 || halfw[a] == dg_align_halfwidth(q_len[a], t_len[a]);
                        if (dg_align_cells(halfw[a]) == kinds[k] && (int)is_final == fin) order[first + fill++] = a;
                    }
                    const uint32_t nk = (uint32_t)(fill - k0);
                    if (!nk) continue;
                    std::stable_sort(order.begin() + first + k0, order.begin() + first + fill,
                                     [&](uint32_t x, uint32_t y) { return q_len[x] > q_len[y]; });
                    HIPCHK(c, hipMemcpyAsync((uint32_t *)didx.p + first + k0, order.data() + first + k0, (size_t)nk * 4, hipMemcpyHostToDevice, s));
                    ap.idx = (const uint32_t *)didx.p + first + k0; ap.n = nk; ap.first_pass = fin ? 0u : 1u;
                    if (local) launch_align_band<true>(kinds[k], nk, s, ap);
                    else launch_align_band<false>(kinds[k], nk, s, ap);
                    HIPCHK(c, hipGetLastError());
                }
            }
            HIPCHK(c, hipStreamSynchronize(s));
            if (t_dbg) {
                const double now = std::chrono::duration<double>(std::chrono::steady_clock::now().time_since_epoch()).count();
                fprintf(stderr, "dagcon_align: pass %d, group of %zu pairs, %.1f MB of directions: %.2f ms\n", pass, cnt, rows * 256.0 / 1e6, (now - t_grp) * 1e3);
                t_grp = now;
            }
            first += cnt;
        }
        if (pass == 0) {
            HIPCHK(c, d2h(c, aln_len, dlen.p, (size_t)n * 4));
            std::vector<uint32_t> again;
            for (uint32_t a : todo) if (aln_len[a] == DG_AL_RETRY) again.push_back(a);
            if (t_dbg) fprintf(stderr, "dagcon_align: %zu of %u pairs go to the full band\n", again.size(), n);
            todo.swap(again);
        }
    }
    HIPCHK(c, d2h(c, aln_len, dlen.p, (size_t)n * 4));
    uint32_t dropped = 0;
    for (uint32_t a = 0; a < n; a++) {
        if ((uint64_t)aln_len[a] > (uint64_t)q_len[a] + t_len[a]) return fail(c, DAGCON_ERR_INTERNAL, "pair %u: alignment longer than its room", a);
        dropped += aln_len[a] == 0 && (q_len[a] || t_len[a]);
    }
    c->h_ends.resize((size_t)n * 4);
    if (local) HIPCHK(c, d2h(c, c->h_ends.data(), dend.p, (size_t)n * 16));
    else
        for (uint32_t a = 0; a < n; a++) {
            const bool ok = aln_len[a] != 0;
            uint32_t *e = &c->h_ends[(size_t)a * 4];
            e[0] = 0; e[1] = ok ? q_len[a] : 0u; e[2] = 0; e[3] = ok ? t_len[a] : 0u;
        }
    c->align_n = n;
    c->align_dropped = dropped;
    *out_bytes_ret = out_bytes;
    return DAGCON_OK;
}

int dagcon_align(dagcon_ctx *ctx, uint32_t n, const uint64_t *q_off, const uint32_t *q_len,
                 const uint64_t *t_off, const uint32_t *t_len, const char *q_blob, uint64_t q_bytes,
                 const char *t_blob, uint64_t t_bytes, const uint64_t *out_off, char *qaln, char *taln,
                 uint32_t *aln_len) {
    if (!ctx) return DAGCON_ERR_INVALID_ARG;
    Ctx *c = reinterpret_cast<Ctx *>(ctx);
    c->align_n = 0;
    if (n == 0) return DAGCON_OK;
    if (!q_off || !q_len || !t_off || !t_len || !q_blob || !t_blob || !out_off || !qaln || !taln || !aln_len)
        return fail(c, DAGCON_ERR_INVALID_ARG, "NULL argument");
    uint64_t out_bytes = 0;
    int r = align_device(c, n, q_off, q_len, t_off, t_len, q_blob, q_bytes, t_blob, t_bytes, out_off, aln_len, &out_bytes);
    if (r != DAGCON_OK) return r;
    HIPCHK(c, d2h(c, qaln, c->d_al[7].p, out_bytes));
    HIPCHK(c, d2h(c, taln, c->d_al[8].p, out_bytes));
    return DAGCON_OK;
}

int dagcon_align_ends(dagcon_ctx *ctx, uint32_t n, uint32_t *q_begin, uint32_t *q_end, uint32_t *t_begin, uint32_t *t_end) {
    if (!ctx) return DAGCON_ERR_INVALID_ARG;
    Ctx *c = reinterpret_cast<Ctx *>(ctx);
    if (n != c->align_n) return fail(c, DAGCON_ERR_INVALID_ARG, "dagcon_align_ends: %u pairs asked, the last alignment had %u", n, c->align_n);
    if (n && (!q_begin || !q_end || !t_begin || !t_end)) return fail(c, DAGCON_ERR_INVALID_ARG, "NULL argument");
    for (uint32_t a = 0; a < n; a++) {
        const uint32_t *e = &c->h_ends[(size_t)a * 4];
        q_begin[a] = e[0]; q_end[a] = e[1]; t_begin[a] = e[2]; t_end[a] = e[3];
    }
    return DAGCON_OK;
}

extern "C++" {
template <int C, int R>
static void launch_panels(hipStream_t s, const DgPanelParams &pp) {
    constexpr int per_wave = R * 64 * (C <= 4 ? 1 : 2);
    constexpr int WPB = per_wave >= 65536 ? 1 : 65536 / per_wave > 4 ? 4 : 65536 / per_wave;
    hipLaunchKernelGGL((k_align_panel<C, R, WPB>), dim3((pp.n + WPB - 1) / WPB), dim3(64 * WPB), 0, s, pp);
}
}

int dagcon_align_panels(dagcon_ctx *ctx, uint32_t n, const uint64_t *q_off, const uint32_t *q_len, const uint64_t *t_off,
                        const uint32_t *t_len, const char *q_blob, uint64_t q_bytes, const char *t_blob, uint64_t t_bytes,
                        const uint64_t *panel_begin, const uint32_t *panel_t_len, const uint32_t *panel_q_len,
                        const uint64_t *out_off, char *qaln, char *taln, uint32_t *aln_len, int32_t *panel_dist) {
    if (!ctx) return DAGCON_ERR_INVALID_ARG;
    Ctx *c = reinterpret_cast<Ctx *>(ctx);
    c->align_dropped = 0;
    if (n == 0) return DAGCON_OK;
    if (!q_off || !q_len || !t_off || !t_len || !q_blob || !t_blob || !panel_begin || !out_off || !qaln || !taln || !aln_len)
        return fail(c, DAGCON_ERR_INVALID_ARG, "NULL argument");
    const uint64_t np = panel_begin[n];
    if (np && (!panel_t_len || !panel_q_len)) return fail(c, DAGCON_ERR_INVALID_ARG, "NULL argument");
    if (np > 0xFFFFFFF0ull) return fail(c, DAGCON_ERR_UNSUPPORTED, "too many panels");
    HIPCHK(c, hipSetDevice(c->device));
    std::vector<uint64_t> p_qoff(np), p_toff(np), p_scr(np);
    std::vector<uint32_t> kept, cls[9];
    std::vector<uint8_t> drop(n, 0);
    uint64_t out_bytes = 0, scr_bytes = 0;
    uint32_t dropped = 0;
    for (uint32_t a = 0; a < n; a++) {
        if (q_off[a] > q_bytes || q_len[a] > q_bytes - q_off[a] || t_off[a] > t_bytes || t_len[a] > t_bytes - t_off[a])
            return fail(c, DAGCON_ERR_INVALID_ARG, "pair %u runs past its blob", a);
        if ((uint64_t)q_len[a] + t_len[a] > 0x7FFFFFF0ull) return fail(c, DAGCON_ERR_UNSUPPORTED, "pair %u too long", a);
// ... 766 lines not shown
```

### pbdagcon_amd/csrc/k_bestpath.hip.h

```cpp
#pragma once
#include <hip/hip_runtime.h>
#include <float.h>
#include <type_traits>
#include "dagcon_dev.h"

#define DG_TT_TEN 1.0e30f
__global__ __launch_bounds__(256) void k_bp_terms(DgParams p) {
    const uint32_t t = blockIdx.x;
    if (dg_failed(p) || dg_tskip(p, t)) return;
    const uint64_t nb = p.node_base[t];
    const uint32_t N = p.n_nodes[t];
    const int32_t *cov = p.cov + p.bbv_base[t];
    const DgNode *nd = p.nodes + nb;
    for (uint32_t v = blockIdx.y * 256 + threadIdx.x; v < N; v += gridDim.y * 256) {
        const uint4 h = *reinterpret_cast<const uint4 *>(&nd[v]);
        const uint4 h2 = *(reinterpret_cast<const uint4 *>(&nd[v]) + 1);
        float tt;
        if (((h.y >> 8) & DG_NF_BACKBONE) && (int)h.z == 1) tt = DG_TT_TEN;
        else tt = (float)cov[(int)h2.w] * 0.5f;
        p.bp_tt[nb + v] = tt;
        p.score[nb + v] = make_float2(0.0f, 0.0f);
        p.best[nb + v] = -1;
    }
}

#ifndef DG_SR
#define DG_SR 256
#define DG_BOUT 6
#endif
#define DG_BR 64
#define DG_WR 256
#define DG_BSTK 64
#define DG_BDEF 32
#define DG_BFAR 192
#define DG_BL_HBM  0x40000000
#define DG_BL_DONE 0x20000000

struct DgBpShared {
    int stag[DG_SR];
    float sval[DG_SR];
    int tag[DG_BR];
    int lens[DG_BR];
    int out_dst[DG_BR * DG_BOUT];
    float out_w[DG_BR * DG_BOUT];
    int stk[DG_BSTK];
    int def_v[DG_BDEF], def_b[DG_BDEF];
    int rbest[DG_BR];
    float rscore[DG_BR];
};
struct DgBpSharedB {
    float svalb[DG_SR], rscoreb[DG_BR];
};
struct DgWalkShared {
    unsigned char wbuf[64];
    int wtag[DG_WR], wbest[DG_WR], wbase[DG_WR], wweight[DG_WR];
};
struct DgWalkSharedS : DgWalkShared {
    uint32_t sw[64], sb[64];
};

__device__ __forceinline__ bool dg_sup_put(uint32_t *dst, uint32_t w, int32_t d) {
    *dst = (w & 0xffffu) | ((uint32_t)d << 16);
    return w > 0xffffu || (uint32_t)d > 0xffffu;
}

#define DG_BP_PIECES 256
#define DG_BP_NINF (-1.0e9f)
#define DG_BP_ONE 0xFFFFFFFFu
template <bool AB = false>
__device__ __forceinline__ void dg_bp_sweep(DgBpShared &S, const DgNode *nd, int32_t *best, float2 *score,
                                            const uint32_t *pool, const float *tt, const int v_top, const int v_bot,
                                            const int c_top, int32_t *gstk, const int gstk_cap,
                                            const int lane, float &amax, bool &bad, bool &stuck,
                                            const float ctv = 0.0f, const int xid = -1, const float xv = 0.0f,
                                            const bool skip_def = false, float *score_b = nullptr, DgBpSharedB *SB = nullptr) {
    const int dead_mask = (int)DG_NF_DELETED | (skip_def ? (int)DG_NF_DEFER : 0);
    for (int i = lane; i < DG_SR; i += 64) S.stag[i] = -1;
    for (int i = lane; i < DG_BR; i += 64) S.tag[i] = -1;
    if (c_top >= 0 && lane == 0) {
        S.stag[c_top & (DG_SR - 1)] = c_top; S.sval[c_top & (DG_SR - 1)] = ctv;
        if constexpr (AB) SB->svalb[c_top & (DG_SR - 1)] = DG_BP_NINF;
    }

    uint4 r_lo, r_hi, n_lo, n_hi;
    int e_dst[DG_BOUT], e_w[DG_BOUT];
    float e_t[DG_BOUT];
#define DG_LOAD_REC(C, LO, HI)                                                             \
    do {                                                                                    \
        const int v_ = v_top - 64 * (C) - lane;                                             \
        LO = make_uint4(0, 0, 0, 0); HI = make_uint4(0, 0, 0, 0);                           \
        if (v_ >= v_bot) {                                                                      \
            LO = *reinterpret_cast<const uint4 *>(&nd[v_]);                                 \
            HI = *(reinterpret_cast<const uint4 *>(&nd[v_]) + 1);                           \
        }                                                                                   \
    } while (0)
#define DG_LOAD_ENT(LO, HI)                                                                 \
    do {                                                                                    \
        const int ol_ = (int)((LO).x & 0xffffu);                                            \
        _Pragma("unroll") for (int k_ = 0; k_ < DG_BOUT; k_++) {                            \
            e_dst[k_] = 0; e_w[k_] = 0;                                                     \
            if (ol_ <= DG_BOUT && k_ < ol_) { e_dst[k_] = (int)pool[(HI).x + 2 * k_]; e_w[k_] = (int)pool[(HI).x + 2 * k_ + 1]; } \
        }                                                                                   \
    } while (0)
#define DG_LOAD_TT()                                                                        \
    do {                                                                                    \
        _Pragma("unroll") for (int k_ = 0; k_ < DG_BOUT; k_++) e_t[k_] = tt[e_dst[k_]];     \
    } while (0)
#define DG_WRITE_CHUNK(C, LO)                                                               \
    do {                                                                                    \
        const int v_ = v_top - 64 * (C) - lane;                                             \
        if (v_ >= v_bot) {                                                                      \
            const int x_ = v_ & (DG_BR - 1);                                                \
            const int ol_ = (int)((LO).x & 0xffffu);                                        \
            int ln_ = (ol_ <= DG_BOUT ? ol_ : DG_BL_HBM) | (int)(((LO).y >> 8) & 0xffu) << 16; \
            S.tag[x_] = v_;                                                                 \
            S.lens[x_] = ln_;                                                               \
            if (ol_ <= DG_BOUT) {                                                           \
                _Pragma("unroll") for (int k_ = 0; k_ < DG_BOUT; k_++) {                    \
                    S.out_dst[x_ * DG_BOUT + k_] = e_dst[k_];                               \
                    S.out_w[x_ * DG_BOUT + k_] = e_t[k_] == DG_TT_TEN ? -10.0f : (float)e_w[k_] - e_t[k_];  \
                }                                                                           \
            }                                                                               \
        }                                                                                   \
    } while (0)

    const int n_chunks = (v_top - v_bot + 1 + 63) / 64;
    DG_LOAD_REC(0, r_lo, r_hi);
    DG_LOAD_ENT(r_lo, r_hi);
    DG_LOAD_TT();
    DG_WRITE_CHUNK(0, r_lo);
    DG_LOAD_REC(1, r_lo, r_hi);
    DG_LOAD_ENT(r_lo, r_hi);
    DG_LOAD_REC(2, n_lo, n_hi);
    DG_LOAD_TT();

    unsigned long long guard = 0;
    const unsigned long long guard_max = 64ull * (unsigned long long)(v_top - v_bot + 1) + 1000000ull;

    int ndef = 0;
    auto collect = [&](const int x, const int q0) -> int {
        const bool in = lane < ndef;
        const int wv = in ? S.def_v[lane] : 0, wb = in ? S.def_b[lane] : -1;
        const unsigned long long hit = __ballot(in && wb == x);
        if (!hit) return 0;
        const unsigned long long below = (1ull << lane) - 1ull;
        if ((hit >> lane) & 1ull) {
            const int q = q0 + __popcll(hit & below);
            if (q < DG_BSTK) S.stk[q] = wv; else gstk[q - DG_BSTK] = wv;
        } else if (in) {
            const unsigned long long stay = __ballot(in) & ~hit;
            const int k = __popcll(stay & below);
            S.def_v[k] = wv; S.def_b[k] = wb;
        }
        ndef -= __popcll(hit);
        __builtin_amdgcn_fence(__ATOMIC_SEQ_CST, "workgroup");
        return __popcll(hit);
    };
    bool tt_due = false;
    for (int c = 0; c < n_chunks && !bad; c++) {
        if (c > 0) {
            DG_WRITE_CHUNK(c, r_lo);
            r_lo = n_lo; r_hi = n_hi;
            DG_LOAD_ENT(r_lo, r_hi);
            DG_LOAD_REC(c + 2, n_lo, n_hi);
            tt_due = true;
        }
        const int v_hi = v_top - 64 * c;
        const int v_lo = v_hi - 63 < v_bot ? v_bot : v_hi - 63;

        const int el = lane < DG_BOUT ? lane : 0;
        unsigned long long live;
        {
            const int vl = v_hi - lane;
            const int lnl = vl >= v_lo ? S.lens[vl & (DG_BR - 1)] : (int)DG_BL_DONE;
            live = __ballot(!(lnl & DG_BL_DONE) && !((lnl >> 16) & dead_mask));
        }
        int pf_ln = 0, pf_d = 0;
        float pf_w = 0.0f;
        if (live) {
            const int x0 = (v_hi - (__ffsll((long long)live) - 1)) & (DG_BR - 1);
            pf_ln = S.lens[x0]; pf_d = S.out_dst[x0 * DG_BOUT + el]; pf_w = S.out_w[x0 * DG_BOUT + el];
        }
        while (live && !bad) {
            const int v = v_hi - (__ffsll((long long)live) - 1);
            live &= live - 1ull;
            int woken = 0;
            {
                const int xs = v & (DG_BR - 1);
                const int ln = __builtin_amdgcn_readfirstlane(pf_ln);
                const int d = pf_d;
                const float w = pf_w;
                if (live) {
                    const int xn = (v_hi - (__ffsll((long long)live) - 1)) & (DG_BR - 1);
                    pf_ln = S.lens[xn]; pf_d = S.out_dst[xn * DG_BOUT + el]; pf_w = S.out_w[xn * DG_BOUT + el];
                }
                if (ln & DG_BL_DONE) continue;
                if (!(ln & DG_BL_HBM)) {
                    const int ol = ln & 0xffff;
                    const int y = d & (DG_SR - 1);
                    const int stg = S.stag[y];
                    const float ns = w + S.sval[y];
                    float nsb = 0.0f;
                    if constexpr (AB) nsb = w + SB->svalb[y];
                    const bool ok = lane >= ol || stg == d;
                    if (__all(ok)) {
                        float mx = 0.0f, mxb = 0.0f;
                        int bd = -1;
                        if (ol > 0) {
                            mx = __int_as_float(__builtin_amdgcn_readlane(__float_as_int(ns), 0));
                            bd = __builtin_amdgcn_readlane(d, 0);
                            if constexpr (AB) mxb = __int_as_float(__builtin_amdgcn_readlane(__float_as_int(nsb), 0));
                            for (int i = 1; i < ol; i++) {
                                const float xsx = __int_as_float(__builtin_amdgcn_readlane(__float_as_int(ns), i));
                                if (xsx > mx) { mx = xsx; bd = __builtin_amdgcn_readlane(d, i); }
                                if constexpr (AB) mxb = fmaxf(mxb, __int_as_float(__builtin_amdgcn_readlane(__float_as_int(nsb), i)));
                            }
                        }
                        if (lane == 0) {
                            S.stag[v & (DG_SR - 1)] = v;
                            S.sval[v & (DG_SR - 1)] = mx;
                            S.rscore[xs] = mx; S.rbest[xs] = bd;
                            S.lens[xs] = ln | DG_BL_DONE;
                            if constexpr (AB) { SB->svalb[v & (DG_SR - 1)] = mxb; SB->rscoreb[xs] = mxb; }
                        }
                        if (mx > 0.5f * DG_BP_NINF) amax = fmaxf(amax, fabsf(mx));
                        if constexpr (AB) if (mxb > 0.5f * DG_BP_NINF) amax = fmaxf(amax, fabsf(mxb));
                        if (ndef) woken = collect(v, 0);
                        if (!woken) continue;
                    }
                }
            }
            int sp = 1 + woken;
            while (sp > 0) {
                if (++guard > guard_max) { bad = true; stuck = true; break; }
                int n;
                if (sp == 1) n = v;
                else if (sp - 2 < DG_BSTK) n = __builtin_amdgcn_readfirstlane(S.stk[sp - 2]);
                else n = __builtin_amdgcn_readfirstlane(gstk[sp - 2 - DG_BSTK]);
                const int x = n & (DG_BR - 1);
                const int tg_ = S.tag[x], ln_ = S.lens[x];
                const bool in_ring = __builtin_amdgcn_readfirstlane(tg_) == n;
                int lens;
                if (in_ring) lens = __builtin_amdgcn_readfirstlane(ln_);
                else {
                    const uint4 lo = *reinterpret_cast<const uint4 *>(&nd[n]);
                    const float fin = score[n].y;
                    lens = __builtin_amdgcn_readfirstlane((int)DG_BL_HBM | (int)((lo.y >> 8) & 0xffu) << 16 |
                                                          (fin >= 1.0f ? (int)DG_BL_DONE : 0));
                }
                if ((lens & DG_BL_DONE) || ((lens >> 16) & DG_NF_DELETED)) { sp--; continue; }
                int out_len = lens & 0xffff;
                const bool hbm = (lens & DG_BL_HBM) != 0;
                uint32_t out_off = 0;
                if (hbm) {
                    const DgNode nn = nd[n];
                    out_off = __builtin_amdgcn_readfirstlane(nn.out_off);
                    out_len = __builtin_amdgcn_readfirstlane((int)nn.out_len);
                }
                float mx = 0.0f, mxb = 0.0f;
                int bd = -1;
                bool again = false;
                for (int e0 = 0; e0 < out_len; e0 += 64) {
                    const int idx = e0 + lane;
                    const bool valid = idx < out_len;
                    int d = 0;
                    float w = 0.0f;
                    if (valid) {
                        if (!hbm) { d = S.out_dst[x * DG_BOUT + idx]; w = S.out_w[x * DG_BOUT + idx]; }
                        else {
                            d = (int)pool[out_off + 2 * idx];
                            const float td = tt[d];
                            w = td == DG_TT_TEN ? -10.0f : (float)(int)pool[out_off + 2 * idx + 1] - td;
                        }
                    }
                    const int y = d & (DG_SR - 1);
                    const int stg = S.stag[y];
                    float sc = S.sval[y], scb = 0.0f;
                    if constexpr (AB) scb = SB->svalb[y];
                    bool have = valid && stg == d;
                    if (valid && !have) {
                        const int yd = d & (DG_BR - 1);
                        if (d == c_top) { have = true; sc = ctv; if constexpr (AB) scb = DG_BP_NINF; }
                        else if (d == xid) { have = true; sc = xv; if constexpr (AB) scb = 0.0f; }
                        else if (S.tag[yd] == d && (S.lens[yd] & DG_BL_DONE) && d >= v_lo) {
                            have = true; sc = S.rscore[yd];
                            if constexpr (AB) scb = SB->rscoreb[yd];
                        } else {
                            const float2 sg = score[d];
                            if (sg.y >= 1.0f) {
                                have = true; sc = (sg.y == 2.0f && xv < 0.5f * DG_BP_NINF) ? xv : sg.x;
                                if constexpr (AB) scb = sg.y == 2.0f ? sg.x : score_b[d];
                            }
                        }
                    }
                    const unsigned long long miss = __ballot(valid && !have);
                    if (miss) {
                        const unsigned long long far = __ballot(valid && !have && d < v - DG_BFAR);
                        if (far && ndef + sp <= DG_BDEF) {
                            const int dfar = __builtin_amdgcn_readlane(d, __ffsll((long long)far) - 1);
                            int above = dfar;
                            for (int q = sp - 1; q >= 0; q--) {
                                int who;
                                if (q == 0) who = v;
                                else if (q - 1 < DG_BSTK) who = __builtin_amdgcn_readfirstlane(S.stk[q - 1]);
                                else who = __builtin_amdgcn_readfirstlane(gstk[q - 1 - DG_BSTK]);
                                if (lane == 0) { S.def_v[ndef] = who; S.def_b[ndef] = above; }
                                ndef++;
                                above = who;
                            }
                            __builtin_amdgcn_fence(__ATOMIC_SEQ_CST, "workgroup");
                            sp = 0;
                            again = true;
                            break;
                        }
                        if (sp + __popcll(miss) > DG_BSTK + gstk_cap) { bad = true; break; }
                        if (valid && !have) {
                            const int si = sp - 1 + __popcll(miss & ((1ull << lane) - 1ull));
                            if (si < DG_BSTK) S.stk[si] = d; else gstk[si - DG_BSTK] = d;
                        }
                        sp += __popcll(miss);
                        again = true;
                        break;
                    }
                    const float ns = w + sc;
                    const int cnt = out_len - e0 < 64 ? out_len - e0 : 64;
// ... 883 lines not shown
```

### pbdagcon_amd/csrc/k_build.hip.h

```cpp
#pragma once
#include <hip/hip_runtime.h>
#include "dagcon_dev.h"

#define DG_WAVE 64
#ifndef DG_LPW
#define DG_LPW 8u
#endif

__device__ __forceinline__ bool dg_failed(const DgParams &p) {
    return __hip_atomic_load(&p.st->err_flags, __ATOMIC_RELAXED, __HIP_MEMORY_SCOPE_AGENT) != 0;
}
__device__ __forceinline__ void dg_fail(const DgParams &p, uint32_t bit) {
    atomicOr(&p.st->err_flags, bit);
}
__device__ __forceinline__ void dg_fail_target(const DgParams &p, uint32_t t, uint32_t bit) {
    atomicOr(&p.tfail[t], bit);
}
__device__ __forceinline__ bool dg_tskip(const DgParams &p, uint32_t t) {
    return !p.tactive[t] || __hip_atomic_load(&p.tfail[t], __ATOMIC_RELAXED, __HIP_MEMORY_SCOPE_AGENT) != 0;
}
__device__ __forceinline__ bool dg_askip(const DgParams &p, uint32_t a) {
    return !(p.flags & DG_F_A1_ONLY) && __hip_atomic_load(&p.tfail[p.aln_tgt[a]], __ATOMIC_RELAXED, __HIP_MEMORY_SCOPE_AGENT) != 0;
}
__device__ __forceinline__ void dg_fail_aln(const DgParams &p, uint32_t a, uint32_t bit) {
    if (p.flags & DG_F_A1_ONLY) dg_fail(p, bit);
    else dg_fail_target(p, p.aln_tgt[a], bit);
    p.st->bad_aln = a;
}

#define DG_COL(qb, tb) ((uint16_t)((uint16_t)(qb) | ((uint16_t)(tb) << 8)))
#define DG_Q(c) ((uint8_t)((c) & 0xff))
#define DG_T(c) ((uint8_t)((c) >> 8))
#define DG_NW 64u
#define DG_NW_BIG 512u
#define DG_REDO 0xFFFFFFFFu

__device__ inline void dg_finish_alignment(const DgParams &p, uint32_t a, uint16_t *buf, uint32_t m) {
    const uint32_t trim = p.trim;
    uint32_t lbases = 0, rbases = 0, lo = 0, hi = m;
    uint32_t start = p.aln_start[a];
    while (lbases < trim && lo < m) {
        if (DG_T(buf[lo++]) != DG_GAP) lbases++;
    }
    while (rbases < trim && hi > lo) {
        if (DG_T(buf[--hi]) != DG_GAP) rbases++;
    }
    start += lbases;
    const bool graph = !(p.flags & DG_F_A1_ONLY);
    uint32_t t_idx = 0, r = 0;
    uint32_t *Cm = nullptr;
    if (graph) {
        t_idx = p.aln_tgt[a];
        if (p.tactive[t_idx]) {
            const uint64_t ab = p.aln_begin[t_idx];
            r = (uint32_t)(a - ab);
            Cm = p.matC + p.matc_base[t_idx] + (uint64_t)r * p.matc_stride[t_idx];
        }
    }
    const uint32_t tlen = graph ? p.tlen[t_idx] : 0xFFFFFFFFu;
    uint32_t n_ins = 0, n_del = 0, adv = 0, run = 0;
    bool conf = start >= 1;
    uint32_t i = lo;
#define DG_FIN_COL(c, ci_)                                                                \
    do {                                                                                  \
        const uint8_t qb_ = DG_Q(c), tb_ = DG_T(c);                                       \
        if (qb_ == tb_ || qb_ == DG_GAP) {                                                \
            if (Cm && conf && ((start + adv) & ((1u << p.emit_shift) - 1u)) == 0 && start + adv <= tlen + 1) \
                ck[(start + adv) >> p.emit_shift] = ci_ - run;                            \
            if (run) { if (Cm && conf && start + adv <= tlen + 1) Cm[start + adv] = run; run = 0; } \
            adv++; n_del += (qb_ != tb_);                                                 \
            if ((uint64_t)start - 1 + adv > (uint64_t)tlen) conf = false;                 \
        } else if (tb_ == DG_GAP) { n_ins++; run++; }                                     \
    } while (0)
    uint32_t *ck = p.ckpt + p.ck_base[a];
    while (i < hi && (i & 7u)) { const uint16_t c = buf[i]; DG_FIN_COL(c, i); i++; }
    while (i + 8 <= hi) {
        const uint4 v = *reinterpret_cast<const uint4 *>(buf + i);
        const uint32_t w4[4] = {v.x, v.y, v.z, v.w};
#pragma unroll
        for (int k = 0; k < 4; k++) {
            const uint16_t c0 = (uint16_t)(w4[k] & 0xffffu), c1 = (uint16_t)(w4[k] >> 16);
            DG_FIN_COL(c0, i + 2 * k);
            DG_FIN_COL(c1, i + 2 * k + 1);
        }
        i += 8;
    }
    while (i < hi) { const uint16_t c = buf[i]; DG_FIN_COL(c, i); i++; }
    if (run && Cm && conf && ((start + adv) & ((1u << p.emit_shift) - 1u)) == 0 && start + adv <= tlen + 1)
        ck[(start + adv) >> p.emit_shift] = hi - run;
    if (run && Cm && conf && start + adv <= tlen + 1) Cm[start + adv] = run;
#undef DG_FIN_COL
    p.n_lo[a] = lo; p.n_hi[a] = hi; p.n_start[a] = start;
    p.n_ins[a] = n_ins; p.n_del[a] = n_del;
    atomicAdd(&p.st->n_columns, (unsigned long long)(hi - lo));
    if (graph && hi > lo && !conf) dg_fail_aln(p, a, DG_E_NONCONF);
}

#ifndef DG_NCH
#define DG_NCH 512u
#endif
#define DG_CH_NONE 0xFFFFFFFFu

__device__ __forceinline__ bool dg_match_col(uint8_t qb, uint8_t tb) { return qb == tb && qb != DG_GAP && qb != '.'; }

__device__ inline uint32_t dg_chunk_start(const uint8_t *q, const uint8_t *t, uint32_t len, uint32_t c) {
    if (c == 0) return 0;
    const uint64_t w0 = (uint64_t)c * DG_NCH;
    if (w0 >= len) return DG_CH_NONE;
    const uint32_t hi = (uint64_t)len < w0 + DG_NCH ? len : (uint32_t)(w0 + DG_NCH);
    for (uint32_t k = (uint32_t)w0; k < hi; k++) {
        const uint8_t b = q[k];
        if (dg_match_col(b, t[k]) && b != q[k - 1] && dg_match_col(q[k - 1], t[k - 1]) && dg_match_col(q[k - 2], t[k - 2]))
            return k;
    }
    return DG_CH_NONE;
}

struct DgChunkRun { uint32_t w, tb; bool dirty, overflow, badchar; };

template <uint32_t NW>
__device__ inline DgChunkRun dg_norm_run(const uint8_t *q, const uint8_t *t, const uint32_t len, const uint32_t k0,
                                         const uint32_t k1, uint16_t *win, uint16_t *out) {
#define DG_W(x) win[(x) & (NW - 1u)]
    DgChunkRun r;
    r.w = 0; r.tb = 0; r.dirty = false; r.overflow = false; r.badchar = false;
    if (k0 >= k1) return r;
    uint32_t badw = 0;
    uint32_t ip = k0, e = 0, i = 0, w = 0, tb = 0, jt = 0, jq = 0;
    uint32_t e_end = 0xFFFFFFFFu;
    uint32_t o0 = 0, o1 = 0, o2 = 0, o3 = 0;
    uint32_t in_done = 0, dirty = 0, overflow = 0;
    for (;;) {
        asm volatile("" : "+v"(in_done), "+v"(dirty));
        if (!in_done && (e - i) + 32u > NW) { overflow = 1; break; }
        if (!in_done) {
            uint32_t take = len - ip;
            if (take > 16u) take = 16u;
            if (ip < k1 && take > k1 - ip) take = k1 - ip;
#define DG_EXPAND(QB, TB)                                                      \
            do {                                                               \
                uint8_t qb_ = (QB), tb_ = (TB);                                \
                if (qb_ == '.') qb_ = DG_GAP;                                  \
                if (tb_ == '.') tb_ = DG_GAP;                                  \
                 \
                                   \
                const bool mm_ = qb_ != tb_ && qb_ != DG_GAP && tb_ != DG_GAP; \
                DG_W(e) = mm_ ? DG_COL(DG_GAP, tb_) : DG_COL(qb_, tb_);        \
                DG_W(e + 1u) = DG_COL(qb_, DG_GAP);                            \
                e += mm_ ? 2u : 1u;                                            \
            } while (0)
            if (take == 16u && (((uintptr_t)(q + ip)) & 15u) == 0) {
                const uint4 qv = *reinterpret_cast<const uint4 *>(q + ip);
                const uint4 tv = *reinterpret_cast<const uint4 *>(t + ip);
                const uint32_t qw[4] = {qv.x, qv.y, qv.z, qv.w}, tw[4] = {tv.x, tv.y, tv.z, tv.w};
#pragma unroll
                for (int k = 0; k < 4; k++) {
                    badw |= ((qw[k] - 0x21212121u) & ~qw[k]) | ((qw[k] + 0x01010101u) | qw[k]);
                    badw |= ((tw[k] - 0x21212121u) & ~tw[k]) | ((tw[k] + 0x01010101u) | tw[k]);
                }
#pragma unroll
                for (int k = 0; k < 16; k++)
                    DG_EXPAND((uint8_t)(qw[k >> 2] >> (8 * (k & 3))), (uint8_t)(tw[k >> 2] >> (8 * (k & 3))));
            } else {
                const uint32_t to_align = (uint32_t)((16u - (((uintptr_t)(q + ip)) & 15u)) & 15u);
                if (to_align && take > to_align) take = to_align;
                for (uint32_t k = 0; k < take; k++) {
                    const uint8_t qb0 = q[ip + k], tb0 = t[ip + k];
                    if (qb0 < 33 || qb0 > 126 || tb0 < 33 || tb0 > 126) badw = 0x80u;
                    DG_EXPAND(qb0, tb0);
                }
            }
#undef DG_EXPAND
            ip += take;
            if (ip == k1) e_end = e;
            if (ip == len) in_done = 1;
        }
        while (i < e && i < e_end) {
            if (i + 1 == e && !in_done) break;
            const uint16_t c = DG_W(i);
            uint8_t qi = DG_Q(c), ti = DG_T(c);
            uint32_t more = 0;
            if (i + 1 < e) {
                if (ti == DG_GAP) {
                    if (jt <= i) jt = i + 1;
                    while (jt < e && DG_T(DG_W(jt)) == DG_GAP) jt++;
                    if (jt < e) {
                        const uint16_t cj = DG_W(jt);
                        if (DG_T(cj) == qi) { ti = qi; DG_W(jt) = DG_COL(DG_Q(cj), DG_GAP); dirty |= (uint32_t)(jt >= e_end); }
                    } else if (!in_done) more = 2;
                }
                if (!more && qi == DG_GAP) {
                    if (jq <= i) jq = i + 1;
                    while (jq < e && DG_Q(DG_W(jq)) == DG_GAP) jq++;
                    if (jq < e) {
                        const uint16_t cj = DG_W(jq);
                        if (DG_Q(cj) == ti) { qi = ti; DG_W(jq) = DG_COL(DG_GAP, DG_T(cj)); dirty |= (uint32_t)(jq >= e_end); }
                    } else if (!in_done) more = 2;
                }
            }
            if (more) { DG_W(i) = DG_COL(qi, ti); break; }
            if (qi != DG_GAP || ti != DG_GAP) {
                o0 = (o0 >> 16) | (o1 << 16); o1 = (o1 >> 16) | (o2 << 16); o2 = (o2 >> 16) | (o3 << 16);
                o3 = (o3 >> 16) | ((uint32_t)DG_COL(qi, ti) << 16);
                w++;
                tb += (ti != DG_GAP);
                if ((w & 7u) == 0) *reinterpret_cast<uint4 *>(out + w - 8) = make_uint4(o0, o1, o2, o3);
            }
            i++;
        }
        if (i == e_end) break;
    }
#undef DG_W
    for (uint32_t k = w & 7u, x = w - (w & 7u); k > 0; k--, x++) {
        const uint32_t sh = 8u - k;
        const uint32_t word = sh >> 1;
        const uint32_t v = word == 0 ? o0 : word == 1 ? o1 : word == 2 ? o2 : o3;
        out[x] = (uint16_t)((sh & 1u) ? v >> 16 : v & 0xffffu);
    }
    r.w = w; r.tb = tb; r.dirty = dirty != 0; r.overflow = overflow != 0; r.badchar = (badw & 0x80808080u) != 0;
    return r;
}

template <uint32_t NW, uint32_t LANES, bool RETRY>
__global__ __launch_bounds__(LANES) void k_norm_chunk(DgParams p) {
    __shared__ uint16_t s_win[LANES * (NW + 2u)];
    const uint32_t g = threadIdx.x * gridDim.x + blockIdx.x;
    if (g >= p.n_chunks) return;
    if (dg_failed(p)) return;
    if (RETRY && p.ch_flag[g] != 2u) return;
    const uint32_t a = p.ch_aln[g];
    if (dg_askip(p, a)) { if (!RETRY) p.ch_flag[g] = 0; return; }
    const uint32_t c = g - p.ch_base[a], nwin = p.ch_base[a + 1] - p.ch_base[a];
    const uint64_t off = p.aln_off[a];
    const uint32_t len = p.aln_len[a];
    const uint8_t *q = p.q + off, *t = p.t + off;
    uint32_t flag = 0;
    DgChunkRun r;
    r.w = 0; r.tb = 0; r.dirty = false; r.overflow = false; r.badchar = false;
    uint32_t k0 = DG_CH_NONE, cn = c + 1;
    uint64_t src = 0;
    if (p.flags & DG_F_RAW) {
        if (c == 0) { k0 = 0; cn = nwin; flag = 1; }
    } else {
        k0 = dg_chunk_start(q, t, len, c);
        if (k0 != DG_CH_NONE) {
            uint16_t *win = s_win + threadIdx.x * (NW + 2u);
            src = (2ull * (off + k0) + 8ull * g + 7ull) & ~7ull;
            for (;;) {
                uint32_t k1 = len;
                for (; cn < nwin; cn++) {
                    const uint32_t s = dg_chunk_start(q, t, len, cn);
                    if (s != DG_CH_NONE) { k1 = s; break; }
                }
                r = dg_norm_run<NW>(q, t, len, k0, k1, win, p.norm_tmp + src);
                if (r.badchar) dg_fail_aln(p, a, DG_E_BADCHAR);
                if (r.overflow) { flag = RETRY ? 1u : 2u; break; }
                if (!r.dirty) break;
                cn++;
                uint32_t k2 = len;
                for (uint32_t x = cn; x < nwin; x++) {
                    const uint32_t s = dg_chunk_start(q, t, len, x);
                    if (s != DG_CH_NONE) { k2 = s; break; }
                }
                const unsigned long long need = (2ull * (k2 - k0) + 15ull) & ~7ull;
                const unsigned long long o = atomicAdd(&p.st->ovf_top, need);
                if (p.tmp_main + o + need > p.tmp_cap) { flag = 1; break; }
                src = p.tmp_main + o;
            }
        }
    }
    p.ch_k0[g] = k0; p.ch_next[g] = cn; p.ch_w[g] = r.w; p.ch_tb[g] = r.tb;
    p.ch_flag[g] = flag; p.ch_src[g] = src;
}

__global__ __launch_bounds__(64) void k_norm_scan(DgParams p) {
    const uint32_t a = blockIdx.x * 64 + threadIdx.x;
    if (a >= p.A) return;
    if (dg_failed(p)) return;
    if (dg_askip(p, a)) return;
    const uint32_t g0 = p.ch_base[a], g1 = p.ch_base[a + 1];
    bool redo = false;
    uint32_t m = 0, tbt = 0;
    for (uint32_t g = g0; g < g1;) {
        if (p.ch_k0[g] == DG_CH_NONE) { p.ch_out[g] = DG_CH_NONE; g++; continue; }
        redo |= p.ch_flag[g] != 0;
        p.ch_out[g] = m; p.ch_adv[g] = tbt;
        m += p.ch_w[g]; tbt += p.ch_tb[g];
        uint32_t nx = g0 + p.ch_next[g];
        if (nx > g1) nx = g1;
        for (uint32_t x = g + 1; x < nx; x++) p.ch_out[x] = DG_CH_NONE;
        g = nx;
    }
    if (redo) { p.n_hi[a] = DG_REDO; return; }
    const uint32_t trim = p.trim;
    uint32_t lbases = 0, rbases = 0, lo = 0, hi = m;
    for (uint32_t g = g0; g < g1 && lbases < trim && lo < m; g++) {
        if (p.ch_out[g] == DG_CH_NONE) continue;
        const uint32_t w = p.ch_w[g], tb = p.ch_tb[g];
        if (lbases + tb < trim) { lo += w; lbases += tb; continue; }
        const uint16_t *src = p.norm_tmp + p.ch_src[g];
        for (uint32_t x = 0; x < w && lbases < trim; x++) {
            if (DG_T(src[x]) != DG_GAP) lbases++;
            lo++;
        }
    }
    for (uint32_t g = g1; g > g0 && rbases < trim && hi > lo;) {
        g--;
        const uint32_t o = p.ch_out[g];
        if (o == DG_CH_NONE) continue;
        const uint32_t tb = p.ch_tb[g];
        if (o >= lo && rbases + tb < trim) { hi = o; rbases += tb; continue; }
        const uint16_t *src = p.norm_tmp + p.ch_src[g];
        while (rbases < trim && hi > lo && hi > o) {
            if (DG_T(src[--hi - o]) != DG_GAP) rbases++;
        }
    }
    p.n_lo[a] = lo; p.n_hi[a] = hi; p.n_start[a] = p.aln_start[a] + lbases; p.n_lb[a] = lbases;
    p.n_ins[a] = 0; p.n_del[a] = 0;
    atomicAdd(&p.st->n_columns, (unsigned long long)(hi - lo));
}

__device__ __forceinline__ uint4 dg_funnel_cols(const uint4 A, const uint4 B, const uint32_t h) {
    const bool w1 = (h >> 1) & 1u, w2 = (h >> 2) & 1u, half = h & 1u;
    const uint32_t u0 = w1 ? A.y : A.x, u1 = w1 ? A.z : A.y, u2 = w1 ? A.w : A.z, u3 = w1 ? B.x : A.w,
                   u4 = w1 ? B.y : B.x, u5 = w1 ? B.z : B.y, u6 = w1 ? B.w : B.z;
    const uint32_t t0 = w2 ? u2 : u0, t1 = w2 ? u3 : u1, t2 = w2 ? u4 : u2, t3 = w2 ? u5 : u3, t4 = w2 ? u6 : u4;
    uint4 r;
    r.x = half ? __builtin_amdgcn_alignbit(t1, t0, 16) : t0;
    r.y = half ? __builtin_amdgcn_alignbit(t2, t1, 16) : t1;
    r.z = half ? __builtin_amdgcn_alignbit(t3, t2, 16) : t2;
    r.w = half ? __builtin_amdgcn_alignbit(t4, t3, 16) : t3;
    return r;
}

__device__ __forceinline__ uint32_t dg_wave_excl(const uint32_t v, const int lane) {
    int incl = (int)v;
    incl += __builtin_amdgcn_update_dpp(0, incl, 0x111, 0xf, 0xf, false);
    incl += __builtin_amdgcn_update_dpp(0, incl, 0x112, 0xf, 0xf, false);
    incl += __builtin_amdgcn_update_dpp(0, incl, 0x114, 0xf, 0xf, false);
    incl += __builtin_amdgcn_update_dpp(0, incl, 0x118, 0xf, 0xf, false);
    incl += __builtin_amdgcn_update_dpp(0, incl, 0x142, 0xa, 0xf, false);
    incl += __builtin_amdgcn_update_dpp(0, incl, 0x143, 0xc, 0xf, false);
    (void)lane;
    return (uint32_t)incl - v;
}

__global__ __launch_bounds__(256) void k_norm_finish2(DgParams p) {
    const uint32_t g = blockIdx.x * 4u + (threadIdx.x >> 6);
    if (g >= p.n_chunks) return;
    if (dg_failed(p)) return;
    const int lane = threadIdx.x & 63;
    const uint32_t a = p.ch_aln[g];
    if (dg_askip(p, a)) return;
    const uint32_t o = p.ch_out[g];
    if (o == DG_CH_NONE) return;
    const uint32_t hi = p.n_hi[a];
    if (hi == DG_REDO) return;
    const uint32_t lo = p.n_lo[a], start = p.n_start[a], lb = p.n_lb[a];
    const uint32_t w = p.ch_w[g], adv0 = p.ch_adv[g];
    const uint16_t *src = p.norm_tmp + p.ch_src[g];
    const uint4 *src4 = reinterpret_cast<const uint4 *>(src);
    uint16_t *dst = p.norm + p.norm_off[a] + o;
    const bool graph = !(p.flags & DG_F_A1_ONLY);
    uint32_t t_idx = 0;
    uint32_t *Cm = nullptr;
    if (graph) {
        t_idx = p.aln_tgt[a];
        if (p.tactive[t_idx]) Cm = p.matC + p.matc_base[t_idx] + (uint64_t)(a - p.aln_begin[t_idx]) * p.matc_stride[t_idx];
    }
    const uint32_t tlen = graph ? p.tlen[t_idx] : 0xFFFFFFFFu;
    uint32_t *ck = p.ckpt + p.ck_base[a];
    const uint32_t ck_mask = (1u << p.emit_shift) - 1u;
    const uint32_t adv_init = adv0 > lb ? adv0 - lb : 0u;
    const uint32_t f0 = lo > o ? lo - o : 0u;
    const uint32_t f1 = hi > o ? (hi - o < w ? hi - o : w) : 0u;
    const bool any = f1 > f0;
    const uint32_t fspan = any ? f1 - f0 : 0u;
#define DG_FIN_CONF(A) (start >= 1u && ((A) == 0u || (uint64_t)start - 1u + (A) <= (uint64_t)tlen))
    const uint32_t h0 = (8u - (o & 7u)) & 7u;
    const uint32_t h = h0 < w ? h0 : w;
    const uint32_t nb = (w - h) / 8u, nvec = (w + 7u) / 8u;
    if ((uint32_t)lane < h) dst[lane] = src[lane];
    { const uint32_t x = h + 8u * nb + (uint32_t)lane; if (lane < 8 && x < w) dst[x] = src[x]; }
    uint4 *dst4 = reinterpret_cast<uint4 *>(dst + h);
    uint32_t adv_tile = adv_init, run_tile = 0, n_ins = 0, n_del = 0;
    for (uint32_t v0 = 0; v0 < nvec; v0 += 64u) {
        const uint32_t vl = v0 + (uint32_t)lane;
        const uint4 pc = vl < nvec ? src4[vl] : make_uint4(0, 0, 0, 0);
        const uint4 pn = vl + 1 < nvec ? src4[vl + 1] : make_uint4(0, 0, 0, 0);
        if (vl < nb) dst4[vl] = dg_funnel_cols(pc, pn, h);
        if (!any || 8u * v0 >= f1) continue;
        uint32_t advm = 0, insm = 0, delm = 0;
#pragma unroll
        for (uint32_t k = 0; k < 8u; k++) {
            const uint32_t wd = ((k >> 1) & 3u) == 0 ? pc.x : ((k >> 1) & 3u) == 1 ? pc.y : ((k >> 1) & 3u) == 2 ? pc.z : pc.w;
            const uint16_t c = (uint16_t)((k & 1u) ? wd >> 16 : wd & 0xffffu);
            const bool inw = 8u * vl + k < 8u * nvec && 8u * vl + k - f0 < fspan;
            const uint8_t qb = DG_Q(c), tb = DG_T(c);
            const bool adv = inw && (qb == tb || qb == DG_GAP);
            advm |= adv ? 1u << k : 0u;
            delm |= (adv && qb != tb) ? 1u << k : 0u;
            insm |= (inw && !adv && tb == DG_GAP) ? 1u << k : 0u;
        }
        const uint32_t nadv = (uint32_t)__popc(advm), nI = (uint32_t)__popc(insm);
        n_ins += nI; n_del += (uint32_t)__popc(delm);
        const uint32_t adv_lane = adv_tile + dg_wave_excl(nadv, lane);
        uint32_t sf = advm ? 1u : 0u;
        uint32_t sv = advm ? (uint32_t)__popc(insm & ~((2u << (31 - __clz((int)advm))) - 1u)) : nI;
#pragma unroll
        for (int d = 1; d < 64; d <<= 1) {
            const uint32_t pf = (uint32_t)__shfl_up((int)sf, d), pv = (uint32_t)__shfl_up((int)sv, d);
            if (lane >= d) { sv = sf ? sv : pv + sv; sf |= pf; }
        }
        uint32_t ef = (uint32_t)__shfl_up((int)sf, 1), ev = (uint32_t)__shfl_up((int)sv, 1);
        if (lane == 0) { ef = 0; ev = 0; }
        uint32_t run = ef ? ev : ev + run_tile;
        const uint32_t lf = (uint32_t)__builtin_amdgcn_readlane((int)sf, 63), lv = (uint32_t)__builtin_amdgcn_readlane((int)sv, 63);
        run_tile = lf ? lv : lv + run_tile;
        adv_tile += (uint32_t)__builtin_amdgcn_readlane((int)(adv_lane - adv_tile + nadv), 63);
        uint32_t adv = adv_lane;
        if (Cm && (advm | insm)) {
#pragma unroll
            for (uint32_t k = 0; k < 8u; k++) {
                if ((advm >> k) & 1u) {
                    const bool conf = DG_FIN_CONF(adv);
                    const uint32_t x = 8u * vl + k;
                    if (conf && ((start + adv) & ck_mask) == 0 && start + adv <= tlen + 1 && !(x == 0 && o > lo))
                        ck[(start + adv) >> p.emit_shift] = o + x - run;
                    if (run && conf && start + adv <= tlen + 1) Cm[start + adv] = run;
                    run = 0;
                    adv++;
                } else if ((insm >> k) & 1u) run++;
            }
        }
    }
    {
        const uint32_t adv = adv_tile, run = run_tile;
        const bool conf = DG_FIN_CONF(adv);
        if (lane == 0) {
            if (any && Cm && conf && ((start + adv) & ck_mask) == 0 && start + adv <= tlen + 1 && (o + f1 < hi || run))
                ck[(start + adv) >> p.emit_shift] = o + f1 - run;
            if (run && Cm && conf && start + adv <= tlen + 1) Cm[start + adv] = run;
            if (graph && any && !conf) dg_fail_aln(p, a, DG_E_NONCONF);
        }
    }
    {
        const uint32_t ti = dg_wave_excl(n_ins, lane) + n_ins, td = dg_wave_excl(n_del, lane) + n_del;
        if (lane == 63) { if (ti) atomicAdd(&p.n_ins[a], ti); if (td) atomicAdd(&p.n_del[a], td); }
    }
#undef DG_FIN_CONF
}

__global__ __launch_bounds__(64) void k_normalize_slow(DgParams p) {
    const uint32_t a = blockIdx.x * 64 + threadIdx.x;
    if (a >= p.A) return;
    if (dg_failed(p)) return;
    if (dg_askip(p, a)) return;
    if (p.n_hi[a] != DG_REDO) return;
    const uint64_t off = p.aln_off[a];
    const uint32_t len = p.aln_len[a];
    const uint8_t *q = p.q + off, *t = p.t + off;
    uint16_t *buf = p.norm + p.norm_off[a];
    const bool raw = (p.flags & DG_F_RAW) != 0;
    uint32_t n = 0;
    for (uint32_t i = 0; i < len; i++) {
        uint8_t qb = q[i], tb = t[i];
        if (qb < 33 || qb > 126 || tb < 33 || tb > 126) dg_fail_aln(p, a, DG_E_BADCHAR);
        if (!raw) {
            if (qb == '.') qb = DG_GAP;
            if (tb == '.') tb = DG_GAP;
            if (qb != tb && qb != DG_GAP && tb != DG_GAP) {
                buf[n++] = DG_COL(DG_GAP, tb);
                buf[n++] = DG_COL(qb, DG_GAP);
                continue;
            }
        }
        buf[n++] = DG_COL(qb, tb);
    }
    uint32_t m = n;
    if (!raw) {
        uint32_t w = 0, jt = 0, jq = 0;
        for (uint32_t i = 0; i < n; i++) {
            uint16_t c = buf[i];
            uint8_t qi = DG_Q(c), ti = DG_T(c);
            if (i + 1 < n) {
                if (ti == DG_GAP) {
                    if (jt <= i) jt = i + 1;
                    while (jt < n && DG_T(buf[jt]) == DG_GAP) jt++;
                    if (jt < n) {
                        uint16_t cj = buf[jt];
                        if (DG_T(cj) == qi) { ti = qi; buf[jt] = DG_COL(DG_Q(cj), DG_GAP); }
                    }
                }
                if (qi == DG_GAP) {
                    if (jq <= i) jq = i + 1;
                    while (jq < n && DG_Q(buf[jq]) == DG_GAP) jq++;
                    if (jq < n) {
                        uint16_t cj = buf[jq];
                        if (DG_Q(cj) == ti) { qi = ti; buf[jq] = DG_COL(DG_GAP, DG_T(cj)); }
                    }
                }
            }
            if (qi != DG_GAP || ti != DG_GAP) buf[w++] = DG_COL(qi, ti);
        }
        m = w;
    }
    dg_finish_alignment(p, a, buf, m);
}

__device__ __forceinline__ uint32_t dg_pool_words(uint32_t tlen, uint32_t n_ins, uint32_t n_del,
                                                  uint32_t k, uint32_t growth_pct, uint32_t *fixed_words) {
    const uint64_t capb = dg_capb(k);
    const uint64_t fixed = 3ull * n_ins + (uint64_t)(tlen + 2) * 3ull * capb;
    const uint64_t spill = 3ull * ((uint64_t)n_ins + n_del + 2ull * k) + 64ull;
    const uint64_t growth = (fixed * growth_pct) / 100ull + spill + 256ull;
    *fixed_words = (uint32_t)fixed;
    const uint64_t tot = fixed + growth;
    return tot > 0xFFFFFFF0ull ? 0xFFFFFFF0u : (uint32_t)tot;
}

__global__ __launch_bounds__(1024) void k_carve(DgParams p) {
    __shared__ unsigned long long s_scan[1024];
    __shared__ unsigned long long s_carry_nodes, s_carry_pool;
    if (dg_failed(p)) return;
    const uint32_t tid = threadIdx.x;
    if (tid == 0) { s_carry_nodes = 0; s_carry_pool = 0; }
    __syncthreads();
    for (uint32_t t0 = 0; t0 < p.T; t0 += 1024) {
        const uint32_t t = t0 + tid;
        unsigned long long nodes = 0, poolw = 0;
        uint32_t fixed_words = 0, ins = 0;
        if (t < p.T && !dg_tskip(p, t)) {
            uint32_t del = 0;
            const uint64_t b = p.aln_begin[t], e = p.aln_begin[t + 1];
            for (uint64_t a = b; a < e; a++) { ins += p.n_ins[a]; del += p.n_del[a]; }
            nodes = (unsigned long long)p.tlen[t] + 2ull + ins;
            poolw = dg_pool_words(p.tlen[t], ins, del, (uint32_t)(e - b), p.growth_pct, &fixed_words);
            if (nodes > DG_MAX_NODES || poolw > 0x3FFFFFFFull) {
                dg_fail_target(p, t, DG_E_TOO_BIG);
                nodes = 0; poolw = 0; fixed_words = 0;
            }
        }
        s_scan[tid] = nodes;
        __syncthreads();
        for (uint32_t o = 1; o < 1024; o <<= 1) {
            unsigned long long v = tid >= o ? s_scan[tid - o] : 0;
            __syncthreads();
            s_scan[tid] += v;
            __syncthreads();
        }
        unsigned long long node_excl = s_scan[tid] - nodes + s_carry_nodes;
        unsigned long long node_tot = s_scan[1023];
        __syncthreads();
        s_scan[tid] = poolw;
        __syncthreads();
        for (uint32_t o = 1; o < 1024; o <<= 1) {
            unsigned long long v = tid >= o ? s_scan[tid - o] : 0;
            __syncthreads();
            s_scan[tid] += v;
            __syncthreads();
        }
        unsigned long long pool_excl = s_scan[tid] - poolw + s_carry_pool;
        unsigned long long pool_tot = s_scan[1023];
        __syncthreads();
        if (t < p.T) {
            p.node_base[t] = node_excl;
            p.n_nodes[t] = (uint32_t)nodes;
            p.pool_base[t] = pool_excl;
            p.pool_size[t] = (uint32_t)poolw;
            p.pool_top[t] = fixed_words;
            p.t_nins[t] = ins;
        }
        if (tid == 0) { s_carry_nodes += node_tot; s_carry_pool += pool_tot; }
        __syncthreads();
    }
    if (tid == 0) {
        p.st->node_need = s_carry_nodes;
        p.st->pool_need = s_carry_pool;
        if (s_carry_nodes > p.node_cap) dg_fail(p, DG_E_NODE_OVF);
        if (s_carry_pool > p.pool_cap) dg_fail(p, DG_E_POOL_OVF);
    }
}

__global__ __launch_bounds__(64) void k_readspan(DgParams p) {
    const uint32_t a = blockIdx.x * 64 + threadIdx.x;
    if (a >= p.A) return;
    if (dg_failed(p)) return;
    const uint32_t t = p.aln_tgt[a];
    uint32_t s = 0, e = 0, lead = 0, trail = 0;
    if (!dg_tskip(p, t)) {
        const uint32_t lo = p.n_lo[a], hi = p.n_hi[a];
        if (hi > lo && hi != DG_REDO) {
            const uint16_t *col = p.norm + p.norm_off[a];
            const uint32_t ins = p.n_ins[a];
            uint32_t i = lo, dels = 0;
            for (; i < hi; i++) {
                const uint8_t qb = DG_Q(col[i]), tb = DG_T(col[i]);
                if (qb == tb) break;
                if (tb == DG_GAP) lead++; else if (qb == DG_GAP) dels++;
            }
            s = p.n_start[a] + dels;
            if (i < hi) {
                uint32_t k = hi, tdels = 0;
                while (k > i + 1) {
                    const uint8_t qb = DG_Q(col[k - 1]), tb = DG_T(col[k - 1]);
                    if (qb == tb) break;
                    if (tb == DG_GAP) trail++; else if (qb == DG_GAP) tdels++;
                    k--;
                }
                e = p.n_start[a] + (hi - lo - ins) - 1u - tdels;
            } else { e = 0; s = 0; }
        }
    }
    p.rd_s[a] = s; p.rd_e[a] = e; p.rd_lead[a] = lead; p.rd_trail[a] = trail;
}

__global__ __launch_bounds__(256) void k_groups(DgParams p) {
    const uint32_t t = blockIdx.x;
    if (dg_failed(p) || dg_tskip(p, t)) return;
    const int lane = threadIdx.x & 63, wave = threadIdx.x >> 6;
    const uint32_t blen = p.tlen[t];
    const uint32_t K = (uint32_t)(p.aln_begin[t + 1] - p.aln_begin[t]);
    uint32_t *col0 = p.matC + p.matc_base[t];
    const uint32_t cstride = p.matc_stride[t];
    uint32_t *gcount = p.gcount + p.bbv_base[t];
    const uint32_t pos0 = (blockIdx.y * 4 + wave) * 8u;
    if (pos0 >= blen + 2) return;
    uint32_t carry[8];
#pragma unroll
    for (int j = 0; j < 8; j++) carry[j] = 0;
    for (uint32_t r0 = 0; r0 < K; r0 += DG_WAVE) {
        const uint32_t r = r0 + lane;
        uint4 *cell = reinterpret_cast<uint4 *>(col0 + (uint64_t)r * cstride + pos0);
        uint4 a = make_uint4(0, 0, 0, 0), b = a;
        if (r < K) { a = cell[0]; b = cell[1]; }
        uint32_t v[8] = {a.x, a.y, a.z, a.w, b.x, b.y, b.z, b.w};
        uint32_t ex[8];
#pragma unroll
        for (int j = 0; j < 8; j++) {
            uint32_t incl = v[j];
            for (int o = 1; o < DG_WAVE; o <<= 1) {
                const uint32_t up = __shfl_up(incl, o);
                if (lane >= o) incl += up;
            }
            ex[j] = carry[j] + incl - v[j];
            carry[j] += __shfl(incl, DG_WAVE - 1);
        }
        if (r < K) {
            cell[0] = make_uint4(ex[0], ex[1], ex[2], ex[3]);
            cell[1] = make_uint4(ex[4], ex[5], ex[6], ex[7]);
        }
    }
#pragma unroll
    for (int j = 0; j < 8; j++)
        if (lane == j && pos0 + j < blen + 2) gcount[pos0 + j] = carry[j];
}

__global__ __launch_bounds__(1024) void k_gscan(DgParams p) {
    __shared__ uint32_t s_scan[1024];
    __shared__ uint32_t s_carry;
    const uint32_t t = blockIdx.x;
    if (dg_failed(p) || dg_tskip(p, t)) return;
    const uint32_t tid = threadIdx.x;
    const uint32_t np = p.tlen[t] + 2;
    const uint64_t bv = p.bbv_base[t];
    if (tid == 0) s_carry = 0;
    __syncthreads();
    for (uint32_t p0 = 0; p0 < np; p0 += 1024) {
        const uint32_t pos = p0 + tid;
        const uint32_t gc = pos < np ? p.gcount[bv + pos] : 0u;
        const uint32_t v = pos < np ? gc + 1u : 0u;
        s_scan[tid] = v;
        __syncthreads();
        for (uint32_t o = 1; o < 1024; o <<= 1) {
            uint32_t x = tid >= o ? s_scan[tid - o] : 0;
            __syncthreads();
            s_scan[tid] += x;
            __syncthreads();
        }
        const uint32_t excl = s_scan[tid] - v + s_carry;
        const uint32_t tot = s_scan[1023];
        __syncthreads();
        if (pos < np) { p.gbase[bv + pos] = excl; p.bid[bv + pos] = excl + gc; }
        if (tid == 0) s_carry += tot;
        __syncthreads();
    }
    if (tid == 0 && s_carry != p.n_nodes[t]) dg_fail_target(p, t, DG_E_INTERNAL);
}

#define DG_CELL_DUP 0x1FFFFFEu
#define DG_EDONE 0xFFFFFFFFu
#define DG_EF_BB 1u
#define DG_EF_OWN 2u
__device__ __forceinline__ uint32_t dg_emit_fold(unsigned long long em, const uint32_t key, const uint32_t first, const uint32_t pos,
                                                 DgNode *ndt, uint32_t *pool, uint32_t *n_out, const int lane) {
    uint32_t victim = 0;
    *n_out = 0;
    while (em & (em - 1ull)) {
        const int f = __ffsll((long long)em) - 1;
        const uint32_t kf = (uint32_t)__builtin_amdgcn_readlane((int)key, f);
        const unsigned long long same = __ballot(key == kf);
        em &= ~same;
        const uint32_t n = (uint32_t)__popcll(same);
        if (n < 2 || !((same >> lane) & 1ull)) continue;
        const uint32_t nins = (key & 0xFF0000u) ? 3u : (key & 0xFF00u) ? 2u : 1u;
        if (lane == f) {
            *n_out = n;
            for (uint32_t k = 0; k < nins; k++) {
                const uint32_t id = first + k, rk = id - pos;
                reinterpret_cast<DgNode *>(reinterpret_cast<char *>(ndt) + (id << 5))->weight = (int32_t)n;
                pool[3u * rk + 1u] = n;
            }
        } else {
            victim = 1;
            for (uint32_t k = 0; k < nins; k++) {
                const uint32_t base = (key >> (8u * (nins - 1u - k))) & 0xFFu;
                *reinterpret_cast<uint2 *>(reinterpret_cast<char *>(ndt) + ((first + k) << 5)) = make_uint2(0u, base | (DG_NF_DELETED << 8));
            }
        }
    }
    return victim;
}

__global__ __launch_bounds__(256) void k_gsum(DgParams p) {
    const uint32_t t = blockIdx.x;
    if (dg_failed(p) || dg_tskip(p, t)) return;
    const uint32_t pos = blockIdx.y * 256u + threadIdx.x;
    if (pos >= p.tlen[t] + 2u) return;
    const uint32_t K = (uint32_t)(p.aln_begin[t + 1] - p.aln_begin[t]);
    const uint32_t *col = p.matC + p.matc_base[t] + pos;
    const uint32_t stride = p.matc_stride[t];
    uint32_t sum = 0;
    for (uint32_t r = 0; r < K; r++) sum += col[(uint64_t)r * stride];
    p.gcount[p.bbv_base[t] + pos] = sum;
}

#ifndef DG_EB
#define DG_EB 8
#endif
#ifndef DG_ERPW
#define DG_ERPW 64
#endif
#ifndef DG_ECOLS
#define DG_ECOLS 40u
#define DG_ECOLS_STRIDE 42u
#define DG_ENEED 16u
#endif
__global__ __launch_bounds__(64) void k_emit(DgParams p) {
    __shared__ uint32_t s_D[DG_EB * 64];
    __shared__ uint16_t s_col[64 * DG_ECOLS_STRIDE];
    if (dg_failed(p)) return;
    const uint32_t t = blockIdx.x;
    if (dg_tskip(p, t)) return;
    const int lane = threadIdx.x;
    uint16_t *colw = s_col + lane * DG_ECOLS_STRIDE;
    const uint64_t ab = p.aln_begin[t];
    const uint32_t K = (uint32_t)(p.aln_begin[t + 1] - ab);
    const uint32_t r = blockIdx.y * DG_ERPW + lane;
    if (blockIdx.y * DG_ERPW >= K) return;
    const bool idle = r >= K || lane >= DG_ERPW;
    const uint32_t a = (uint32_t)(ab + (idle ? 0 : r));
    const uint32_t blen = p.tlen[t];
    const uint32_t exitpos = blen + 1;
    if ((blockIdx.z << p.emit_shift) > exitpos) return;
    const uint64_t nb = p.node_base[t];
    const uint64_t bv = p.bbv_base[t];
    const uint32_t *bid = p.bid + bv, *gbase = p.gbase + bv;
    uint32_t *Am = p.matA + p.mat_base[t];
    uint32_t *Dm = p.matD + p.mat_base[t];
    const uint32_t *Cm = p.matC + p.matc_base[t] + (uint64_t)(idle ? 0 : r) * p.matc_stride[t];
    uint32_t *pool = p.pool + p.pool_base[t];
    DgNode *ndt = p.nodes + nb;
#define DG_EPW(OFF) (*reinterpret_cast<uint32_t *>(reinterpret_cast<char *>(pool) + (((uint32_t)(OFF)) << 2)))
#define DG_ECELL(M, POS) (*reinterpret_cast<uint32_t *>(reinterpret_cast<char *>((M) + (uint64_t)(POS) * K) + (r << 2)))
    const uint16_t *buf = p.norm + p.norm_off[a];
    const uint32_t lo = idle ? 0 : p.n_lo[a], hi = idle ? 0 : p.n_hi[a];
    uint32_t bbpos = idle ? DG_EDONE : p.n_start[a];
    uint32_t prev = 0;
    uint32_t prev_pos = 0;
    uint32_t fl = DG_EF_BB | DG_EF_OWN;
    uint32_t i = lo;
    const uint32_t P0 = blockIdx.z << p.emit_shift, P1 = P0 + (1u << p.emit_shift);
    const bool rvalid = !idle;
    bool pfx_entry = false;
    if (!idle) {
        if (bbpos >= P1) bbpos = DG_EDONE;
        else if (bbpos < P0) {
            const uint32_t ck = p.ckpt[p.ck_base[a] + blockIdx.z];
            if (ck == DG_CK_NONE || ck >= hi) bbpos = DG_EDONE;
            else {
                i = ck; bbpos = P0; fl = DG_EF_BB;
                uint32_t x = ck, d = 0;
                while (x > lo) {
                    const uint16_t c = buf[--x];
                    const uint8_t qb = DG_Q(c), tb = DG_T(c);
                    if (qb == tb) { prev_pos = P0 - 1u - d; prev = bid[prev_pos]; break; }
                    if (qb == DG_GAP) { d++; continue; }
                    if (tb == DG_GAP) {
                        prev_pos = P0 - d;
                        if (p.emit_scan) pfx_entry = true;
                        else {
                            const uint32_t c1 = r + 1 < K ? Cm[p.matc_stride[t] + prev_pos] : p.gcount[bv + prev_pos];
                            prev = gbase[prev_pos] + c1 - 1u;
                        }
                        fl = 0;
                        break;
                    }
                }
            }
        }
    }
    if (p.emit_scan) {
        for (unsigned long long m = __ballot(pfx_entry); m; m = __ballot(pfx_entry)) {
            const uint32_t pp = (uint32_t)__builtin_amdgcn_readlane((int)prev_pos, __ffsll((long long)m) - 1);
            const uint32_t x = rvalid ? Cm[pp] : 0u;
            const uint32_t e = dg_wave_excl(x, lane);
            if (pfx_entry && prev_pos == pp) { prev = gbase[pp] + e + x - 1u; pfx_entry = false; }
        }
    }
    uint32_t c_base = 0x80000000u;
#define DG_STAGE(I)                                                                         \
    do {                                                                                    \
        c_base = (I) & ~7u;                                                                 \
        const uint4 *src_ = reinterpret_cast<const uint4 *>(buf + c_base);                  \
        uint4 v_[DG_ECOLS / 8];                                                             \
        _Pragma("unroll") for (int k_ = 0; k_ < (int)(DG_ECOLS / 8); k_++)                  \
            v_[k_] = (c_base + 8u * k_ < hi) ? src_[k_] : make_uint4(0, 0, 0, 0);           \
        _Pragma("unroll") for (int k_ = 0; k_ < (int)(DG_ECOLS / 8); k_++) {                \
            uint32_t *dst_ = reinterpret_cast<uint32_t *>(colw) + 4 * k_;                   \
            dst_[0] = v_[k_].x; dst_[1] = v_[k_].y; dst_[2] = v_[k_].z; dst_[3] = v_[k_].w; \
        }                                                                                   \
    } while (0)
#define DG_COLUMN(I, OUT)                                                                   \
    do {                                                                                    \
        if ((I) - c_base >= DG_ECOLS) DG_STAGE(I);                                          \
        OUT = colw[(I) - c_base];                                                           \
    } while (0)
#define DG_DEPART(NXT)                                                       \
    do {                                                                     \
        if (!(fl & DG_EF_OWN)) break;                                        \
        if (fl & DG_EF_BB) {                                                 \
            if (prev_pos >= pos0) s_D[(prev_pos - pos0) * 64 + lane] = (NXT) + 1u;   \
            else DG_ECELL(Dm, prev_pos) = (NXT) + 1u;                \
        } else {                                                             \
            const uint32_t _rk = prev - prev_pos;                            \
            DG_EPW(3u * _rk) = (NXT);                                        \
            DG_EPW(3u * _rk + 1u) = 1u;                                      \
        }                                                                    \
    } while (0)

    uint32_t pos0 = P0;
    while (pos0 < P1 && (pos0 <= blen || (!__all(bbpos == DG_EDONE) && pos0 <= blen + 2u * DG_EB))) {
        uint32_t bidv[DG_EB];
        {
            const uint4 *bp = reinterpret_cast<const uint4 *>(bid + pos0);
#pragma unroll
            for (int k = 0; k < DG_EB / 4; k++) {
                const uint4 v = bp[k];
                bidv[4 * k] = v.x; bidv[4 * k + 1] = v.y; bidv[4 * k + 2] = v.z; bidv[4 * k + 3] = v.w;
            }
        }
        uint32_t gbv[DG_EB], cmv[DG_EB];
        {
            const uint4 *gp = reinterpret_cast<const uint4 *>(gbase + pos0);
#pragma unroll
            for (int k = 0; k < DG_EB / 4; k++) {
                const uint4 v = gp[k];
                gbv[4 * k] = v.x; gbv[4 * k + 1] = v.y; gbv[4 * k + 2] = v.z; gbv[4 * k + 3] = v.w;
            }
            const uint4 *cp = reinterpret_cast<const uint4 *>(Cm + pos0);
#pragma unroll
            for (int k = 0; k < DG_EB / 4; k++) {
                const uint4 v = cp[k];
                cmv[4 * k] = v.x; cmv[4 * k + 1] = v.y; cmv[4 * k + 2] = v.z; cmv[4 * k + 3] = v.w;
            }
        }
        if (p.emit_scan) {
#pragma unroll
            for (int j = 0; j < DG_EB; j++) {
                const uint32_t x = rvalid ? cmv[j] : 0u;
                cmv[j] = __ballot(x != 0u) ? dg_wave_excl(x, lane) : 0u;
            }
        }
        if (bbpos != DG_EDONE && i < hi && (i - c_base) + DG_ENEED > DG_ECOLS) DG_STAGE(i);
        uint32_t acell[DG_EB];
#pragma unroll
        for (int j = 0; j < DG_EB; j++) { acell[j] = 0; s_D[j * 64 + lane] = 0; }
        uint32_t exit_val = 0;
#pragma unroll
        for (int j = 0; j < DG_EB; j++) {
            const uint32_t pos = pos0 + j;
            uint32_t f_apos = 0, f_key = 0, f_first = 0;
            asm volatile("" : "+v"(fl));
            if (bbpos == pos && pos < P1) {
                uint32_t ins_id = 0;
                uint32_t kacc = 0;
                uint16_t c = 0;
                f_apos = prev_pos;
                const bool f_anc_ok = fl == (DG_EF_BB | DG_EF_OWN) && pos - prev_pos < 16u;
                for (;;) {
                    if (i < hi) DG_COLUMN(i, c);
                    const uint8_t qb = DG_Q(c), tb = DG_T(c);
                    if (i >= hi || qb == tb || qb == DG_GAP) break;
                    if (tb == DG_GAP) {
                        if (!ins_id) { ins_id = gbv[j] + cmv[j]; f_first = ins_id; }
                        kacc = (kacc << 8) | qb;
                        const uint32_t id = ins_id++;
                        const uint32_t rk = id - bbpos;
                        DgNode nd;
                        nd.out_len = 1; nd.in_len = 1; nd.base = qb; nd.flags = 0; nd.pad = 0;
                        nd.weight = 1; nd.pending = 1;
                        nd.out_off = 3u * rk; nd.in_off = 3u * rk + 2u; nd.out_cap = 1; nd.in_cap = 1;
                        nd.bbpos = (int32_t)bbpos;
                        *reinterpret_cast<DgNode *>(reinterpret_cast<char *>(ndt) + (id << 5)) = nd;
                        DG_EPW(3u * rk + 2u) = prev;
                        DG_DEPART(id);
                        prev = id; prev_pos = bbpos; fl = DG_EF_OWN;
                    }
                    i++;
                }
                if (i >= hi) {
                    exit_val = (fl & DG_EF_OWN) ? prev + 1u : 0u;
                    const uint32_t ex = bid[exitpos];
                    DG_DEPART(ex);
                    bbpos = DG_EDONE;
                } else {
                    const uint8_t qb = DG_Q(c), tb = DG_T(c);
                    if (qb == tb) {
                        const uint32_t cur = bidv[j];
                        acell[j] = ((uint32_t)tb << 25) | (prev + 1u);
                        if (f_anc_ok && kacc != 0u && kacc < (1u << 24)) f_key = kacc | ((pos - f_apos) << 24);
                        DG_DEPART(cur);
                        prev = cur; prev_pos = bbpos; fl = DG_EF_BB | DG_EF_OWN;
                    } else {
                        acell[j] = ((uint32_t)tb << 25) | DG_CELL_DEL;
                    }
                    bbpos++;
                    i++;
                }
            }
            if (p.fold) {
                const unsigned long long em = __ballot(f_key != 0u);
                if (em & (em - 1ull)) {
                    uint32_t fn;
                    const uint32_t vic = dg_emit_fold(em, f_key, f_first, pos, ndt, pool, &fn, lane);
                    if (vic | fn) {
                        const uint32_t dv = vic ? 0u : (f_first + 1u) | ((fn - 1u) << 25);
                        if (f_apos >= pos0) s_D[(f_apos - pos0) * 64 + lane] = dv;
                        if (f_apos < pos0 || f_apos == 0u) DG_ECELL(Dm, f_apos) = dv;
                        if (vic) acell[j] = (acell[j] & 0xFE000000u) | DG_CELL_DUP;
                    }
                }
            }
        }
        if (r < K && lane < DG_ERPW) {
#pragma unroll
            for (int j = 0; j < DG_EB; j++) {
                const uint32_t pos = pos0 + j;
                if (pos <= blen && pos >= P0 && pos < P1) {
                    DG_ECELL(Am, pos) = acell[j];
                    const uint32_t dv = s_D[j * 64 + lane];
                    if (pos > 0 || dv) DG_ECELL(Dm, pos) = dv;
                }
            }
            if (exit_val) DG_ECELL(Am, exitpos) = exit_val;
        }
        pos0 += DG_EB;
    }
    {
        const bool ahead = bbpos != DG_EDONE && (fl & DG_EF_OWN);
        uint32_t q = bbpos, nxt = 0;
        bool found = false, pfx_next = false;
        if (ahead) {
            while (i < hi) {
                const uint16_t c = buf[i];
                const uint8_t qb = DG_Q(c), tb = DG_T(c);
                if (qb == tb) { nxt = bid[q]; found = true; break; }
                if (qb == DG_GAP) { q++; i++; continue; }
                if (tb == DG_GAP) {
                    if (p.emit_scan) pfx_next = true; else nxt = gbase[q] + Cm[q];
                    found = true; break;
                }
                i++;
            }
        }
        if (p.emit_scan) {
            for (unsigned long long m = __ballot(pfx_next); m; m = __ballot(pfx_next)) {
                const uint32_t pp = (uint32_t)__builtin_amdgcn_readlane((int)q, __ffsll((long long)m) - 1);
                const uint32_t x = rvalid ? Cm[pp] : 0u;
                const uint32_t e = dg_wave_excl(x, lane);
                if (pfx_next && q == pp) { nxt = gbase[pp] + e; pfx_next = false; }
            }
        }
        if (ahead) {
            if (!found) {
                nxt = bid[exitpos];
                Am[(uint64_t)exitpos * K + r] = prev + 1u;
            }
            const uint32_t pos0 = 0xFFFFFFFFu;
            DG_DEPART(nxt);
        }
    }
#undef DG_EPW
#undef DG_ECELL
#undef DG_DEPART
#undef DG_COLUMN
#undef DG_STAGE
}

__device__ __forceinline__ int dg_lds_find(volatile int32_t *vals, int n, int x, int lane) {
    for (int b = 0; b < n; b += DG_WAVE) {
        int i = b + lane;
        bool hit = (i < n) && (vals[i] == x);
        unsigned long long m = __ballot(hit);
        if (m) return b + (__ffsll((long long)m) - 1);
    }
    return -1;
}

__device__ __forceinline__ uint32_t dg_pool_alloc(const DgParams &p, uint32_t t, uint32_t words, int lane) {
    uint32_t off = 0;
    if (lane == 0) {
        t = (uint32_t)__builtin_amdgcn_readfirstlane((int)t);
        off = atomicAdd(&p.pool_top[t], words);
        if ((uint64_t)off + words > p.pool_size[t]) { dg_fail(p, DG_E_POOL_TGT); p.st->bad_target = t; off = 0xFFFFFFFFu; }
    }
    return (uint32_t)__builtin_amdgcn_readlane((int)off, 0);
}

__device__ __forceinline__ unsigned long long dg_list_row(int32_t val, int32_t extra, int32_t chain, int32_t ulo, int32_t uhi,
                                                          int lane, int32_t &cnt, unsigned long long &cm) {
    cm = __ballot(val == chain);
    const bool uniq = val >= ulo && val < uhi;
    unsigned long long firsts = __ballot(uniq);
    cnt = 1 + extra;
    unsigned long long rem = __ballot(val != 0 && !uniq) & ~cm;
    while (rem) {
// ... 247 lines not shown
```

Baseline: 333.5 million.

## Pack result arrays into one buffer, fuse gcount sum into normalize, skip deleted nodes

Status, tfail, cns_len, n_seg, cns_off and seg_first now sit in one device buffer. That buffer is copied asynchronously into pinned host memory at the end of the pipeline, replacing several synchronous small device-to-host copies with one copy plus host memcpy. The separate k_gsum kernel, which summed matC columns per target, is removed. gcount is instead built with atomicAdd while normalize writes each insertion run, after a memset. The bestpath init kernel now skips the tt computation for deleted nodes. These changes cut launch and copy overhead, at the cost of atomic contention on gcount.

```diff
diff --git a/pbdagcon_amd/csrc/dagcon_api.hip b/pbdagcon_amd/csrc/dagcon_api.hip
--- a/pbdagcon_amd/csrc/dagcon_api.hip
+++ b/pbdagcon_amd/csrc/dagcon_api.hip
@@ -92,7 +92,7 @@
     uint32_t n_chunks = 0;
     uint64_t tmp_main = 0, tmp_cap = 0;
 
-    DevBuf d_tfail, d_q, d_t, d_aln_off, d_aln_len, d_aln_start, d_aln_tgt, d_tlen, d_aln_begin, d_tactive,
+    DevBuf d_q, d_t, d_aln_off, d_aln_len, d_aln_start, d_aln_tgt, d_tlen, d_aln_begin, d_tactive,
         d_bb, d_bb_off, d_mat_base, d_bbv_base, d_matc_base, d_matc_stride;
     DevBuf d_nmis, d_norm_off, d_n_lo, d_n_hi, d_n_start, d_n_ins, d_n_del, d_norm;
     DevBuf d_ch_aln, d_ch_base, d_ch_k0, d_ch_next, d_ch_w, d_ch_tb, d_ch_flag, d_ch_src, d_ch_out, d_ch_adv,
@@ -108,7 +108,13 @@
     DevBuf d_cg[18];
     std::vector<uint8_t> h_cig_bad;
     std::string cig_err;
-    DevBuf d_cns, d_cns_off, d_cns_len, d_seg_first, d_n_seg, d_seg_r0, d_seg_r1, d_st;
+    DevBuf d_cns, d_seg_r0, d_seg_r1;
+    DevBuf d_res;
+    size_t res_tfail = 0, res_cns_len = 0, res_n_seg = 0, res_cns_off = 0, res_seg_first = 0, res_bytes = 0;
+    char *h_res = nullptr;
+    size_t h_res_cap = 0;
+    int32_t *h_seg = nullptr;
+    size_t h_seg_cap = 0;
     DevBuf d_pos_tmp, d_pos_tmp0, d_pos;
     DevBuf d_sup_tmp, d_sup_tmp0, d_sup;
 
@@ -123,7 +129,7 @@
     dagcon_timings tm;
 
     std::vector<uint64_t> r_seg_begin, r_seq_off, r_cns_off, r_seg_first;
-    std::vector<int32_t> r_range0, r_range1, r_tmp0, r_tmp1;
+    std::vector<int32_t> r_range0, r_range1;
     std::vector<uint32_t> r_seq_len, r_cns_len, r_n_seg, r_tfail;
     std::vector<int32_t> r_status;
     char *r_blob = nullptr;
@@ -240,6 +246,30 @@
     return DAGCON_OK;
 }
 
+int res_layout(Ctx *c, uint32_t T) {
+    size_t o = (sizeof(DgStatus) + 255) & ~(size_t)255;
+    c->res_tfail = o; o += ((size_t)T + 2) / 2 * 8;
+    c->res_cns_len = o; o += ((size_t)T + 1) / 2 * 8;
+    c->res_n_seg = o; o += ((size_t)T + 1) / 2 * 8;
+    c->res_cns_off = o; o += (size_t)T * 8;
+    c->res_seg_first = o; o += (size_t)T * 8;
+    c->res_bytes = o;
+    ENSURE(c, c->d_res, o);
+    if (c->h_res_cap < o) {
+        if (c->h_res) (void)hipHostFree(c->h_res);
+        c->h_res = nullptr; c->h_res_cap = 0;
+        const size_t want = o + o / 8 + 4096;
+        HIPCHK(c, hipHostMalloc((void **)&c->h_res, want, hipHostMallocDefault));
+        c->h_res_cap = want;
+    }
+    return DAGCON_OK;
+}
+
+int send_results(Ctx *c) {
+    HIPCHK(c, hipMemcpyAsync(c->h_res, c->d_res.p, c->res_bytes, hipMemcpyDeviceToHost, c->stream));
+    return DAGCON_OK;
+}
+
 void fill_params(Ctx *c, DgParams &p) {
     memset(&p, 0, sizeof p);
     p.q = (const uint8_t *)c->d_q.p; p.t = (const uint8_t *)c->d_t.p;
@@ -249,7 +279,7 @@
     p.aln_tgt = (const uint32_t *)c->d_aln_tgt.p;
     p.tlen = (const uint32_t *)c->d_tlen.p;
     p.aln_begin = (const uint64_t *)c->d_aln_begin.p;
-    p.tactive = (const uint8_t *)c->d_tactive.p; p.tfail = (uint32_t *)c->d_tfail.p;
+    p.tactive = (const uint8_t *)c->d_tactive.p; p.tfail = (uint32_t *)((char *)c->d_res.p + c->res_tfail);
     p.bb = c->have_bb ? (const uint8_t *)c->d_bb.p : nullptr;
     p.bb_off = (const uint64_t *)c->d_bb_off.p;
     p.mat_base = (const uint64_t *)c->d_mat_base.p;
@@ -300,11 +330,11 @@
     p.seg_done = (uint32_t *)c->d_seg_done.p; p.wl_first = (uint32_t *)c->d_wl_first.p;
     p.worklist = (uint32_t *)c->d_worklist.p; p.worklist_cap = c->worklist_cap;
     p.cns = (uint8_t *)c->d_cns.p; p.cns_cap = c->cns_cap;
-    p.cns_off = (uint64_t *)c->d_cns_off.p; p.cns_len = (uint32_t *)c->d_cns_len.p;
-    p.seg_first = (uint64_t *)c->d_seg_first.p; p.n_seg = (uint32_t *)c->d_n_seg.p;
+    p.cns_off = (uint64_t *)((char *)c->d_res.p + c->res_cns_off); p.cns_len = (uint32_t *)((char *)c->d_res.p + c->res_cns_len);
+    p.seg_first = (uint64_t *)((char *)c->d_res.p + c->res_seg_first); p.n_seg = (uint32_t *)((char *)c->d_res.p + c->res_n_seg);
     p.seg_r0 = (int32_t *)c->d_seg_r0.p; p.seg_r1 = (int32_t *)c->d_seg_r1.p;
     p.seg_cap = c->seg_cap;
-    p.st = (DgStatus *)c->d_st.p;
+    p.st = (DgStatus *)c->d_res.p;
     if (c->opts.flags & DAGCON_FLAG_BASE_SUPPORT) {
         p.sup_tmp = (uint32_t *)c->d_sup_tmp.p; p.sup_tmp0 = (uint32_t *)c->d_sup_tmp0.p;
         p.sup_w = (uint16_t *)c->d_sup.p; p.sup_d = p.sup_w + c->cns_cap;
@@ -337,16 +367,15 @@
                           &c->d_node_base, &c->d_n_nodes, &c->d_pool_base, &c->d_pool_size, &c->d_pool_top, &c->d_t_nins, &c->d_cov, &c->d_gcount,
                           &c->d_gbase, &c->d_bid, &c->d_best, &c->d_queue, &c->d_score, &c->d_cns_tmp, &c->d_bp_tt, &c->d_stk, &c->d_cuts,
                           &c->d_cuts_bp, &c->d_bp_stat, &c->d_bp_len, &c->d_rd, &c->d_pro_state, &c->d_sh_cnt, &c->d_wl_first,
-                          &c->d_queue0, &c->d_bp_end, &c->d_bp_ab, &c->d_defer, &c->d_cns_tmp0, &c->d_cns, &c->d_cns_off, &c->d_seg_first,
+                          &c->d_queue0, &c->d_bp_end, &c->d_bp_ab, &c->d_defer, &c->d_cns_tmp0, &c->d_cns,
                           &c->d_seg_r0, &c->d_seg_r1, &c->d_worklist, &c->d_seg_done, &c->d_sup_tmp, &c->d_sup_tmp0, &c->d_sup, &c->d_pos_tmp, &c->d_pos_tmp0, &c->d_pos};
         for (DevBuf *b : work)
             if (b->p && b->cap) HIPCHK(c, hipMemsetAsync(b->p, 0xEE, b->cap, s));
-    }
-    HIPCHK(c, hipMemsetAsync(c->d_st.p, 0, sizeof(DgStatus), s));
-    HIPCHK(c, hipMemsetAsync(c->d_tfail.p, 0, (size_t)c->T * 4 + 4, s));
-    HIPCHK(c, hipMemsetAsync(c->d_cns_len.p, 0, (size_t)c->T * 4, s));
-    HIPCHK(c, hipMemsetAsync(c->d_n_seg.p, 0, (size_t)c->T * 4, s));
+        HIPCHK(c, hipMemsetAsync((char *)c->d_res.p + c->res_cns_off, 0xEE, c->res_bytes - c->res_cns_off, s));
+    }
+    HIPCHK(c, hipMemsetAsync(c->d_res.p, 0, c->res_cns_off, s));
     if (c->matc_cells) HIPCHK(c, hipMemsetAsync(c->d_matC.p, 0, c->matc_cells * 4, s));
+    if (p.emit_scan && c->sum_bb) HIPCHK(c, hipMemsetAsync(c->d_gcount.p, 0, c->sum_bb * 4, s));
     if (c->poison) {
         if ((c->poison & 1) && c->d_matA.p) { HIPCHK(c, hipMemsetAsync(c->d_matA.p, 0xEE, c->d_matA.cap, s)); HIPCHK(c, hipMemsetAsync(c->d_matD.p, 0xEE, c->d_matD.cap, s)); }
         if ((c->poison & 2) && c->d_nodes.p) { HIPCHK(c, hipMemsetAsync(c->d_nodes.p, 0xEE, c->d_nodes.cap, s)); HIPCHK(c, hipMemsetAsync(c->d_pool.p, 0xEE, c->d_pool.cap, s)); }
@@ -360,8 +389,7 @@
     if (c->T > 0) {
         const uint32_t rows4 = (c->max_tlen + 2 + 4 * DG_LPW - 1) / (4 * DG_LPW);
         if (c->gcuts && c->A > 0) hipLaunchKernelGGL(k_readspan, dim3((c->A + 63) / 64), dim3(64), 0, s, p);
-        if (p.emit_scan) hipLaunchKernelGGL(k_gsum, dim3(c->T, (c->max_tlen + 2 + 255) / 256), dim3(256), 0, s, p);
-        else hipLaunchKernelGGL(k_groups, dim3(c->T, (c->max_tlen + 2 + 31) / 32), dim3(256), 0, s, p);
+        if (!p.emit_scan) hipLaunchKernelGGL(k_groups, dim3(c->T, (c->max_tlen + 2 + 31) / 32), dim3(256), 0, s, p);
         hipLaunchKernelGGL(k_gscan, dim3(c->T), dim3(1024), 0, s, p);
         if (c->A > 0)
             hipLaunchKernelGGL(k_emit, dim3(c->T, (c->max_k + DG_ERPW - 1) / DG_ERPW, ((c->max_tlen + 2) >> c->emit_shift) + 1),
@@ -421,7 +449,7 @@
     }
     HIPCHK(c, hipEventRecord(c->ev[4], s));
     HIPCHK(c, hipGetLastError());
-    return DAGCON_OK;
+    return send_results(c);
 }
 
 }
@@ -476,7 +504,7 @@
     }
     for (auto &e : c->ev)
         if (hipEventCreate(&e) != hipSuccess) { delete c; return DAGCON_ERR_HIP; }
-    if (ensure(c, c->d_st, sizeof(DgStatus)) != DAGCON_OK) { delete c; return DAGCON_ERR_WORKSPACE; }
+    if (res_layout(c, 0) != DAGCON_OK) { dagcon_destroy(reinterpret_cast<dagcon_ctx *>(c)); return DAGCON_ERR_WORKSPACE; }
     *out = reinterpret_cast<dagcon_ctx *>(c);
     return DAGCON_OK;
 }
@@ -488,15 +516,17 @@
     if (c->stream) (void)hipStreamSynchronize(c->stream);
     if (c->r_blob) (void)hipHostFree(c->r_blob);
     if (c->r_sup) (void)hipHostFree(c->r_sup);
+    if (c->h_res) (void)hipHostFree(c->h_res);
+    if (c->h_seg) (void)hipHostFree(c->h_seg);
     DevBuf *all[] = {&c->d_q, &c->d_t, &c->d_aln_off, &c->d_aln_len, &c->d_aln_start, &c->d_aln_tgt,
-                     &c->d_tlen, &c->d_aln_begin, &c->d_tactive, &c->d_tfail, &c->d_bb, &c->d_bb_off, &c->d_mat_base, &c->d_matc_base, &c->d_matc_stride,
+                     &c->d_tlen, &c->d_aln_begin, &c->d_tactive, &c->d_res, &c->d_bb, &c->d_bb_off, &c->d_mat_base, &c->d_matc_base, &c->d_matc_stride,
                      &c->d_bbv_base, &c->d_nmis, &c->d_norm_off, &c->d_n_lo, &c->d_n_hi, &c->d_n_start, &c->d_ch_aln, &c->d_ch_base, &c->d_ch_k0, &c->d_ch_next, &c->d_ch_w, &c->d_ch_tb, &c->d_ch_flag, &c->d_ch_src, &c->d_ch_out, &c->d_ch_adv, &c->d_n_lb, &c->d_norm_tmp, &c->d_ckpt, &c->d_ck_base,
                      &c->d_n_ins, &c->d_n_del, &c->d_norm, &c->d_node_base, &c->d_n_nodes,
                      &c->d_pool_base, &c->d_pool_size, &c->d_pool_top, &c->d_t_nins, &c->d_matA, &c->d_matD,
                      &c->d_matC, &c->d_cov, &c->d_gcount, &c->d_gbase, &c->d_bid, &c->d_nodes,
                      &c->d_best, &c->d_queue, &c->d_score, &c->d_cns_tmp, &c->d_bp_tt, &c->d_score_b, &c->d_pool, &c->d_stk, &c->d_cuts, &c->d_cuts_bp, &c->d_bp_stat, &c->d_bp_len, &c->d_worklist, &c->d_rd, &c->d_pro_state, &c->d_sh_cnt, &c->d_seg_done, &c->d_wl_first, &c->d_queue0, &c->d_bp_end, &c->d_bp_ab, &c->d_defer, &c->d_cns_tmp0, &c->d_cns,
-                     &c->d_cns_off, &c->d_cns_len, &c->d_seg_first, &c->d_n_seg, &c->d_seg_r0, &c->d_seg_r1,
-                     &c->d_st, &c->d_sup_tmp, &c->d_sup_tmp0, &c->d_sup, &c->d_pos_tmp, &c->d_pos_tmp0, &c->d_pos};
+                     &c->d_seg_r0, &c->d_seg_r1,
+                     &c->d_sup_tmp, &c->d_sup_tmp0, &c->d_sup, &c->d_pos_tmp, &c->d_pos_tmp0, &c->d_pos};
     for (DevBuf *b : all) free_buf(*b);
     for (DevBuf &b : c->d_al) free_buf(b);
     for (DevBuf &b : c->d_pn) free_buf(b);
@@ -666,13 +696,12 @@
     }
     ENSURE(c, c->d_node_base, (size_t)T * 8); ENSURE(c, c->d_n_nodes, T4);
     ENSURE(c, c->d_pool_base, (size_t)T * 8); ENSURE(c, c->d_pool_size, T4); ENSURE(c, c->d_pool_top, T4);
-    ENSURE(c, c->d_t_nins, T4); ENSURE(c, c->d_tfail, T4 + 4);
+    ENSURE(c, c->d_t_nins, T4);
+    if ((r = res_layout(c, T))) return r;
     ENSURE(c, c->d_matA, c->mat_cells * 4); ENSURE(c, c->d_matD, c->mat_cells * 4);
     ENSURE(c, c->d_matC, c->matc_cells * 4 + 256);
     ENSURE(c, c->d_cov, c->sum_bb * 4); ENSURE(c, c->d_gcount, c->sum_bb * 4);
     ENSURE(c, c->d_gbase, c->sum_bb * 4); ENSURE(c, c->d_bid, c->sum_bb * 4);
-    ENSURE(c, c->d_cns_off, (size_t)T * 8); ENSURE(c, c->d_cns_len, T4);
-    ENSURE(c, c->d_seg_first, (size_t)T * 8); ENSURE(c, c->d_n_seg, T4);
 
     c->node_cap = std::max<uint64_t>(c->node_cap, c->sum_bb + c->sum_len / 7 + 1024);
     c->pool_cap = std::max<uint64_t>(c->pool_cap, 8ull * c->node_cap + 80ull * c->sum_bb + 1024ull * T);
@@ -749,7 +778,7 @@
 
 static int read_status(Ctx *c) {
     HIPCHK(c, hipStreamSynchronize(c->stream));
-    HIPCHK(c, d2h(c, &c->h_st, c->d_st.p, sizeof(DgStatus)));
+    memcpy(&c->h_st, c->h_res, sizeof(DgStatus));
     return DAGCON_OK;
 }
 
@@ -789,7 +818,7 @@
 
     const uint32_t T = c->T;
     c->r_tfail.assign(T, 0); c->r_status.assign(T, DAGCON_OK);
-    if (T) HIPCHK(c, d2h(c, c->r_tfail.data(), c->d_tfail.p, (size_t)T * 4));
+    if (T) memcpy(c->r_tfail.data(), c->h_res + c->res_tfail, (size_t)T * 4);
     uint32_t n_failed = 0;
     c->err.clear();
     for (uint32_t t = 0; t < T; t++) {
@@ -812,7 +841,13 @@
     }
     const uint64_t nseg = c->h_st.seg_top, nb = c->h_st.cns_top;
     c->r_cns_off.assign(T, 0); c->r_cns_len.assign(T, 0); c->r_seg_first.assign(T, 0); c->r_n_seg.assign(T, 0);
-    c->r_tmp0.assign(nseg, 0); c->r_tmp1.assign(nseg, 0);
+    if (c->h_seg_cap < nseg) {
+        if (c->h_seg) (void)hipHostFree(c->h_seg);
+        c->h_seg = nullptr; c->h_seg_cap = 0;
+        const size_t want = (size_t)nseg + (size_t)(nseg / 8) + 1024;
+        HIPCHK(c, hipHostMalloc((void **)&c->h_seg, want * 8, hipHostMallocDefault));
+        c->h_seg_cap = want;
+    }
     if (c->r_blob_cap < nb + 1) {
         if (c->r_blob) (void)hipHostFree(c->r_blob);
         c->r_blob = nullptr; c->r_blob_cap = 0;
@@ -823,15 +858,16 @@
     c->r_blob[nb] = 0;
     const bool full = !(c->opts.flags & (DAGCON_FLAG_STOP_AFTER_BUILD | DAGCON_FLAG_STOP_AFTER_MERGE));
     if (T && full) {
-        HIPCHK(c, d2h(c, c->r_cns_off.data(), c->d_cns_off.p, (size_t)T * 8));
-        HIPCHK(c, d2h(c, c->r_cns_len.data(), c->d_cns_len.p, (size_t)T * 4));
-        HIPCHK(c, d2h(c, c->r_seg_first.data(), c->d_seg_first.p, (size_t)T * 8));
-        HIPCHK(c, d2h(c, c->r_n_seg.data(), c->d_n_seg.p, (size_t)T * 4));
+        memcpy(c->r_cns_off.data(), c->h_res + c->res_cns_off, (size_t)T * 8);
+        memcpy(c->r_cns_len.data(), c->h_res + c->res_cns_len, (size_t)T * 4);
+        memcpy(c->r_seg_first.data(), c->h_res + c->res_seg_first, (size_t)T * 8);
+        memcpy(c->r_n_seg.data(), c->h_res + c->res_n_seg, (size_t)T * 4);
         if (nseg) {
-            HIPCHK(c, d2h(c, c->r_tmp0.data(), c->d_seg_r0.p, nseg * 4));
-            HIPCHK(c, d2h(c, c->r_tmp1.data(), c->d_seg_r1.p, nseg * 4));
-        }
-        if (nb) HIPCHK(c, d2h(c, c->r_blob, c->d_cns.p, nb));
+            HIPCHK(c, hipMemcpyAsync(c->h_seg, c->d_seg_r0.p, nseg * 4, hipMemcpyDeviceToHost, c->stream));
+            HIPCHK(c, hipMemcpyAsync(c->h_seg + nseg, c->d_seg_r1.p, nseg * 4, hipMemcpyDeviceToHost, c->stream));
+        }
+        if (nb) HIPCHK(c, hipMemcpyAsync(c->r_blob, c->d_cns.p, nb, hipMemcpyDeviceToHost, c->stream));
+        HIPCHK(c, hipStreamSynchronize(c->stream));
     }
     c->sup_valid = c->pos_valid = false;
     if (full && (c->opts.flags & DAGCON_FLAG_BASE_SUPPORT)) {
@@ -862,7 +898,7 @@
         if (!full || !c->h_tactive[t] || c->r_tfail[t]) continue;
         for (uint32_t i = 0; i < c->r_n_seg[t]; i++) {
             const uint64_t s = c->r_seg_first[t] + i;
-            const int32_t r0 = c->r_tmp0[s], r1 = c->r_tmp1[s];
+            const int32_t r0 = c->h_seg[s], r1 = c->h_seg[nseg + s];
             c->r_range0.push_back(r0); c->r_range1.push_back(r1);
             c->r_seq_off.push_back(c->r_cns_off[t] + (uint64_t)r0);
             c->r_seq_len.push_back((uint32_t)(r1 - r0));
@@ -918,7 +954,7 @@
     HIPCHK(c, hipSetDevice(c->device));
     HIPCHK(c, hipStreamSynchronize(c->stream));
     DgStatus st;
-    HIPCHK(c, d2h(c, &st, c->d_st.p, sizeof st));
+    HIPCHK(c, d2h(c, &st, c->d_res.p, sizeof st));
     for (int i = 0; i < 16; i++) out8[i] = st.dbg[i];
     return DAGCON_OK;
 }
@@ -980,10 +1016,10 @@
         DgParams p;
         fill_params(c, p);
         p.flags |= DG_F_A1_ONLY;
-        HIPCHK(c, hipMemsetAsync(c->d_st.p, 0, sizeof(DgStatus), c->stream));
-        HIPCHK(c, hipMemsetAsync(c->d_tfail.p, 0, (size_t)c->T * 4 + 4, c->stream));
+        HIPCHK(c, hipMemsetAsync(c->d_res.p, 0, c->res_cns_len, c->stream));
         launch_normalize(c, p);
         HIPCHK(c, hipGetLastError());
+        if ((r = send_results(c))) return r;
         if ((r = read_status(c))) return r;
         if ((c->h_st.err_flags & DG_E_NORM_OVF) && attempt < 3) {
             c->norm_cap = c->h_st.norm_top + 1024;
diff --git a/pbdagcon_amd/csrc/k_bestpath.hip.h b/pbdagcon_amd/csrc/k_bestpath.hip.h
--- a/pbdagcon_amd/csrc/k_bestpath.hip.h
+++ b/pbdagcon_amd/csrc/k_bestpath.hip.h
@@ -14,13 +14,13 @@
     const DgNode *nd = p.nodes + nb;
     for (uint32_t v = blockIdx.y * 256 + threadIdx.x; v < N; v += gridDim.y * 256) {
         const uint4 h = *reinterpret_cast<const uint4 *>(&nd[v]);
-        const uint4 h2 = *(reinterpret_cast<const uint4 *>(&nd[v]) + 1);
+        p.score[nb + v] = make_float2(0.0f, 0.0f);
+        p.best[nb + v] = -1;
+        if ((h.y >> 8) & DG_NF_DELETED) continue;
         float tt;
         if (((h.y >> 8) & DG_NF_BACKBONE) && (int)h.z == 1) tt = DG_TT_TEN;
-        else tt = (float)cov[(int)h2.w] * 0.5f;
+        else tt = (float)cov[(int)(reinterpret_cast<const uint4 *>(&nd[v]) + 1)->w] * 0.5f;
         p.bp_tt[nb + v] = tt;
-        p.score[nb + v] = make_float2(0.0f, 0.0f);
-        p.best[nb + v] = -1;
     }
 }
 
diff --git a/pbdagcon_amd/csrc/k_build.hip.h b/pbdagcon_amd/csrc/k_build.hip.h
--- a/pbdagcon_amd/csrc/k_build.hip.h
+++ b/pbdagcon_amd/csrc/k_build.hip.h
@@ -35,6 +35,12 @@
 #define DG_NW_BIG 512u
 #define DG_REDO 0xFFFFFFFFu
 
+#define DG_PUT_RUN(Cm, Gc, pos, run)                         \
+    do {                                                     \
+        (Cm)[(pos)] = (run);                                 \
+        if (Gc) atomicAdd(&(Gc)[(pos)], (run));              \
+    } while (0)
+
 __device__ inline void dg_finish_alignment(const DgParams &p, uint32_t a, uint16_t *buf, uint32_t m) {
     const uint32_t trim = p.trim;
     uint32_t lbases = 0, rbases = 0, lo = 0, hi = m;
@@ -48,13 +54,14 @@
     start += lbases;
     const bool graph = !(p.flags & DG_F_A1_ONLY);
     uint32_t t_idx = 0, r = 0;
-    uint32_t *Cm = nullptr;
+    uint32_t *Cm = nullptr, *Gc = nullptr;
     if (graph) {
         t_idx = p.aln_tgt[a];
         if (p.tactive[t_idx]) {
             const uint64_t ab = p.aln_begin[t_idx];
             r = (uint32_t)(a - ab);
             Cm = p.matC + p.matc_base[t_idx] + (uint64_t)r * p.matc_stride[t_idx];
+            if (p.emit_scan) Gc = p.gcount + p.bbv_base[t_idx];
         }
     }
     const uint32_t tlen = graph ? p.tlen[t_idx] : 0xFFFFFFFFu;
@@ -67,7 +74,7 @@
         if (qb_ == tb_ || qb_ == DG_GAP) {                                                \
             if (Cm && conf && ((start + adv) & ((1u << p.emit_shift) - 1u)) == 0 && start + adv <= tlen + 1) \
                 ck[(start + adv) >> p.emit_shift] = ci_ - run;                            \
-            if (run) { if (Cm && conf && start + adv <= tlen + 1) Cm[start + adv] = run; run = 0; } \
+            if (run) { if (Cm && conf && start + adv <= tlen + 1) DG_PUT_RUN(Cm, Gc, start + adv, run); run = 0; } \
             adv++; n_del += (qb_ != tb_);                                                 \
             if ((uint64_t)start - 1 + adv > (uint64_t)tlen) conf = false;                 \
         } else if (tb_ == DG_GAP) { n_ins++; run++; }                                     \
@@ -88,7 +95,7 @@
     while (i < hi) { const uint16_t c = buf[i]; DG_FIN_COL(c, i); i++; }
     if (run && Cm && conf && ((start + adv) & ((1u << p.emit_shift) - 1u)) == 0 && start + adv <= tlen + 1)
         ck[(start + adv) >> p.emit_shift] = hi - run;
-    if (run && Cm && conf && start + adv <= tlen + 1) Cm[start + adv] = run;
+    if (run && Cm && conf && start + adv <= tlen + 1) DG_PUT_RUN(Cm, Gc, start + adv, run);
 #undef DG_FIN_COL
     p.n_lo[a] = lo; p.n_hi[a] = hi; p.n_start[a] = start;
     p.n_ins[a] = n_ins; p.n_del[a] = n_del;
@@ -363,10 +370,13 @@
     uint16_t *dst = p.norm + p.norm_off[a] + o;
     const bool graph = !(p.flags & DG_F_A1_ONLY);
     uint32_t t_idx = 0;
-    uint32_t *Cm = nullptr;
+    uint32_t *Cm = nullptr, *Gc = nullptr;
     if (graph) {
         t_idx = p.aln_tgt[a];
-        if (p.tactive[t_idx]) Cm = p.matC + p.matc_base[t_idx] + (uint64_t)(a - p.aln_begin[t_idx]) * p.matc_stride[t_idx];
+        if (p.tactive[t_idx]) {
+            Cm = p.matC + p.matc_base[t_idx] + (uint64_t)(a - p.aln_begin[t_idx]) * p.matc_stride[t_idx];
+            if (p.emit_scan) Gc = p.gcount + p.bbv_base[t_idx];
+        }
     }
     const uint32_t tlen = graph ? p.tlen[t_idx] : 0xFFFFFFFFu;
     uint32_t *ck = p.ckpt + p.ck_base[a];
@@ -427,7 +437,7 @@
                     const uint32_t x = 8u * vl + k;
                     if (conf && ((start + adv) & ck_mask) == 0 && start + adv <= tlen + 1 && !(x == 0 && o > lo))
                         ck[(start + adv) >> p.emit_shift] = o + x - run;
-                    if (run && conf && start + adv <= tlen + 1) Cm[start + adv] = run;
+                    if (run && conf && start + adv <= tlen + 1) DG_PUT_RUN(Cm, Gc, start + adv, run);
                     run = 0;
                     adv++;
                 } else if ((insm >> k) & 1u) run++;
@@ -440,7 +450,7 @@
         if (lane == 0) {
             if (any && Cm && conf && ((start + adv) & ck_mask) == 0 && start + adv <= tlen + 1 && (o + f1 < hi || run))
                 ck[(start + adv) >> p.emit_shift] = o + f1 - run;
-            if (run && Cm && conf && start + adv <= tlen + 1) Cm[start + adv] = run;
+            if (run && Cm && conf && start + adv <= tlen + 1) DG_PUT_RUN(Cm, Gc, start + adv, run);
             if (graph && any && !conf) dg_fail_aln(p, a, DG_E_NONCONF);
         }
     }
@@ -720,19 +730,6 @@
         }
     }
     return victim;
-}
-
-__global__ __launch_bounds__(256) void k_gsum(DgParams p) {
-    const uint32_t t = blockIdx.x;
-    if (dg_failed(p) || dg_tskip(p, t)) return;
-    const uint32_t pos = blockIdx.y * 256u + threadIdx.x;
-    if (pos >= p.tlen[t] + 2u) return;
-    const uint32_t K = (uint32_t)(p.aln_begin[t + 1] - p.aln_begin[t]);
-    const uint32_t *col = p.matC + p.matc_base[t] + pos;
-    const uint32_t stride = p.matc_stride[t];
-    uint32_t sum = 0;
-    for (uint32_t r = 0; r < K; r++) sum += col[(uint64_t)r * stride];
-    p.gcount[p.bbv_base[t] + pos] = sum;
 }
 
 #ifndef DG_EB
```

New measurement: 322.3 million. 0.966x the previous value.
